# Jellyman750/Linear_Programming_Solver_LPR381

Hardware: AMD Instinct MI355X
Metric: simplex pivots/sec on dense m×n tableau; B&B nodes/sec at 1/2/4/8 GPUs (higher is better)
Workload: dtype f64

## Files before the change

### include/lpx.h

```cpp
#ifndef LPX_H
#define LPX_H

#include <stdint.h>

#ifdef __cplusplus
extern "C" {
#endif

#define LPX_ABI_VERSION 1

enum {
    LPX_OPTIMAL    = 0,
    LPX_UNBOUNDED  = 1,
    LPX_INFEASIBLE = 2,
    LPX_ITER_LIMIT = 3,
    LPX_RUNNING    = 4,
    LPX_CUTOFF     = 5,
    LPX_CUT_INTEGER     = 0,
    LPX_CUT_INCOMPLETE  = 10,
    LPX_CUT_ERROR       = 11,
    LPX_CUT_NOT_OPTIMAL = 12,
    LPX_EINVAL     = -1,
    LPX_EDEVICE    = -2,
    LPX_ENOMEM     = -3,
    LPX_E_GE_PRESENT      = -10,
    LPX_E_NEG_RHS         = -11,
    LPX_E_REVISED_PRECOND = -12,
    LPX_E_SINGULAR        = -13,
    LPX_E_KNAP_SHAPE      = -14,
    LPX_E_UNKNOWN_ALGO    = -15,
    LPX_E_PARSE           = -16
};

typedef void (*lpx_pivot_cb)(void* user, int iter, int row, int col);

typedef struct lpx_stats {
    int64_t pivots;
    int64_t launches;
    double  loop_ms;
    double  h2d_ms;
    double  d2h_ms;
    double  update_ms_sum;
    int64_t update_launches;
    int64_t fdf_pivots;
    int64_t cleanup_pivots;
} lpx_stats;

typedef struct lpx_run_opts {
    double eps;
    double ratio_tol;
    int    max_iter;
    int    fdf_guard;
    int    cleanup;
    int    batch;
    int    use_graph;
    int    profile;
    int    resident;
} lpx_run_opts;

void lpx_default_opts(lpx_run_opts* o, int dual);

int         lpx_abi_version(void);
int         lpx_device_count(void);
int         lpx_init(int device);
int         lpx_last_error(char* buf, int len);
int         lpx_device_name(char* buf, int len);

#define LPX_COMM_ID_BYTES 128
int lpx_comm_unique_id(uint8_t* id );
int lpx_comm_init(int rank, int world, const uint8_t* id);
int lpx_comm_init_tcp(int rank, int world, const char* host, int port);
int lpx_comm_allreduce_max(double* vals, int count);
int lpx_comm_info(int* rank, int* world, int64_t* allreduces, double* allreduce_ms, int* rccl_version);
int lpx_comm_destroy(void);

typedef struct lpx_tableau lpx_tableau;

int  lpx_tableau_create(int R, int C, lpx_tableau** out);
void lpx_tableau_destroy(lpx_tableau* t);
int  lpx_tableau_upload(lpx_tableau* t, const double* T, const int32_t* basis );
int  lpx_tableau_download(lpx_tableau* t, double* T, int32_t* basis );
int  lpx_tableau_snapshot(lpx_tableau* t);
int  lpx_tableau_restore(lpx_tableau* t);
int  lpx_tableau_device_ptr(lpx_tableau* t, void** dptr, int* ld);
int  lpx_tableau_trace(lpx_tableau* t, int32_t* trace , int cap, int* n);
int  lpx_tableau_shape(const lpx_tableau* t, int* R, int* C, int* ld);
int  lpx_tableau_set_shape(lpx_tableau* t, int R, int C);


int lpx_primal_run(lpx_tableau* t, const lpx_run_opts* o, lpx_pivot_cb cb, void* user, lpx_stats* st);

int lpx_dual_run(lpx_tableau* t, const lpx_run_opts* o, lpx_pivot_cb cb, void* user, lpx_stats* st);

int lpx_forced_pivots_run(lpx_tableau* t, const int32_t* rows, const int32_t* cols, int count,
                          double thresh, int32_t* chosen, const lpx_run_opts* o, lpx_stats* st);

int lpx_tableau_solution(lpx_tableau* t, int nvars, double* x, double* z);

int lpx_tableau_build_node(lpx_tableau* node, const lpx_tableau* root, int ncuts, const int32_t* var,
                           const double* coef, const double* zero, const double* rhs);

int lpx_tableau_build_nodes(lpx_tableau** nodes, const lpx_tableau* root, int count, const int32_t* cut_off,
                            const int32_t* var, const double* coef, const double* zero, const double* rhs);

int lpx_tableau_build_child(lpx_tableau* child, lpx_tableau* parent, int var, int row_of_var, int is_ge, double bound);
int lpx_tableau_basis(lpx_tableau* t, int32_t* basis );
int lpx_tableau_solution2(lpx_tableau* t, int nvars, double* x, double* z, int32_t* basis_out );
int lpx_multi_solution(lpx_tableau** ts, int count, int nvars, double* x, double* z, int32_t* basis_out, int basis_stride);
typedef struct lpx_store lpx_store;
int  lpx_store_create(int Rcap, int Ccap, lpx_store** out);
void lpx_store_destroy(lpx_store* s);
int  lpx_store_save(lpx_store* s, lpx_tableau* t, int* slot_out);
int  lpx_store_release(lpx_store* s, int slot);
int  lpx_store_save_multi(lpx_store** stores, lpx_tableau** ts, int count, int* slots);
int  lpx_tableau_build_child_from_store(lpx_tableau* child, lpx_store* s, int slot, int var, int row_of_var,
                                        int is_ge, double bound);

int  lpx_tableau_build_children_from_store(lpx_tableau** children, lpx_store** stores, const int* slots, int count,
                                           const int32_t* var, const int32_t* row_of_var, const int32_t* is_ge, const double* bound);

int lpx_multi_run(lpx_tableau** ts, const int* dual, int count, const lpx_run_opts* primal_opts,
                  const lpx_run_opts* dual_opts, int* statuses, lpx_stats* stats );

int lpx_multi_run_some(lpx_tableau** ts, const int* dual, int count, const lpx_run_opts* primal_opts,
                       const lpx_run_opts* dual_opts, int* statuses, lpx_stats* stats , int min_active);

#define LPX_ASYNC_SLOTS 4
int lpx_multi_run_begin(int slot, lpx_tableau** ts, const int* dual, int count, const lpx_run_opts* primal_opts,
                        const lpx_run_opts* dual_opts, int steps);
int lpx_multi_run_end(int slot, int* statuses, lpx_stats* stats );

int lpx_primal_tableau(double* T, int R, int C, int32_t* basis, double eps, int max_iter,
                       lpx_pivot_cb cb, void* user, lpx_stats* st);
int lpx_dual_tableau(double* T, int R, int C, int32_t* basis, double eps, double ratio_tol,
                     int fdf_guard, int max_iter, int cleanup,
                     lpx_pivot_cb cb, void* user, lpx_stats* st);

typedef struct lpx_revised lpx_revised;
int  lpx_revised_create(int m, int n, const double* A, const double* c, const double* b, lpx_revised** out);
void lpx_revised_destroy(lpx_revised* r);
int  lpx_revised_run(lpx_revised* r, const lpx_run_opts* o, lpx_pivot_cb cb, void* user, lpx_stats* st);
int  lpx_revised_result(lpx_revised* r, int32_t* Bidx, int32_t* Nidx, double* xB, double* z);
int  lpx_revised_binv(lpx_revised* r, double* Binv );
int  lpx_revised_iteration_view(lpx_revised* r, double* rc, double* d);
int  lpx_revised_refactor(lpx_revised* r);
int  lpx_revised_set_refactor(lpx_revised* r, int every);
int  lpx_revised_set_refactor_mode(lpx_revised* r, int mode);
int  lpx_revised_set_drift_policy(lpx_revised* r, int check_every, double tol);
int  lpx_revised_residual(lpx_revised* r, double* rel , double* abs_ );
int  lpx_revised_refactor_stats(lpx_revised* r, int* refactors, int* fast_steps, int* fast_fallbacks, double* last_residual,
                                double* gemm_ms, int* gemm_calls);
int  lpx_revised_profile(lpx_revised* r, int iters, double* us , int* measured);
int  lpx_invert(const double* M, int n, double* inv);
int  lpx_invert_blocked(const double* M, int n, double* inv, double* ms);
int  lpx_revised_trace(lpx_revised* r, int32_t* trace , int cap, int* n);
int  lpx_revised_solve(const double* A, int m, int n, const double* c, const double* b,
                       int32_t* Bidx, int32_t* Nidx, double* xB, double* z,
                       double eps, int max_iter, lpx_pivot_cb cb, void* user, lpx_stats* st);

typedef struct lpx_knapsack lpx_knapsack;
int  lpx_knapsack_create(const double* profit, const double* weight, int n, double cap, lpx_knapsack** out);
void lpx_knapsack_destroy(lpx_knapsack* k);
int  lpx_knapsack_order(lpx_knapsack* k, int32_t* order );
int  lpx_knapsack_relax_batch(lpx_knapsack* k, int count, const int32_t* off, const int32_t* fix_idx,
                              const int8_t* fix_val, double* profit, double* weight, int32_t* frac_idx,
                              double* frac_val);
int  lpx_knapsack_relax_batch2(lpx_knapsack* k, int count, const int32_t* off, const int32_t* fix_idx,
                               const int8_t* fix_val, double* profit, double* weight, int32_t* frac_idx,
                               double* frac_val);
int  lpx_knapsack_has_prefix(lpx_knapsack* k);
int  lpx_knapsack_expand_batch(lpx_knapsack* k, int count, const int64_t* parent, const int32_t* item, const int8_t* val,
                               int64_t* child, double* profit, double* weight, int32_t* frac_idx, double* frac_val);
int  lpx_knapsack_expand_begin(lpx_knapsack* k, int count, const int64_t* parent, const int32_t* item, const int8_t* val, int64_t* child);
int  lpx_knapsack_expand_finish(lpx_knapsack* k, double* profit, double* weight, int32_t* frac_idx, double* frac_val);
int  lpx_knapsack_node_list(lpx_knapsack* k, int64_t node, int32_t* idx, int8_t* val, int cap, int* depth);

enum { LPX_MAX = 0, LPX_MIN = 1 };
enum { LPX_LE = 0, LPX_GE = 1, LPX_EQ = 2 };

typedef struct lpx_problem {
    int sense, n, m;
    const double* c;
    const double* A;
    const int32_t* rel;
    const double* b;
} lpx_problem;

typedef struct lpx_solve_opts {
    int max_iter;
    int batch;
    int render_iterations;
    int dual_flags;
    int bnb_mode;
    int bnb_search;
    int concurrent_nodes;
    int rank, world;
    int64_t max_nodes;
    void (*allreduce_max)(void* user, double* vals, int count);
    void* allreduce_user;
    void (*text_cb)(void* user, const char* text, const uint8_t* highlight, int R, int C);
    void* text_user;
    int bnb_dive;
} lpx_solve_opts;

typedef struct lpx_result {
    int status;
    int has_solution;
    double optimal_value;
    int n; double* x;
    int R, C; double* T;
    int32_t* basis;
    int n_pivots; int32_t* trace;
    char* report; char* summary;
    int64_t lp_solves, nodes;
    int n_log; int32_t* node_log;
    double* node_z;
    double aux[4];
    lpx_stats stats;
    int n_cuts; double* cuts;
} lpx_result;

void lpx_default_solve_opts(lpx_solve_opts* o);
int  lpx_solve(const lpx_problem* p, const char* algorithm, const lpx_solve_opts* o, lpx_result* out);
void lpx_result_free(lpx_result* r);

typedef struct lpx_parsed { int sense, n, m; double* c; double* A; int32_t* rel; double* b; int ragged; } lpx_parsed;
int  lpx_parse_text(const char* text, lpx_parsed* out);
void lpx_parsed_free(lpx_parsed* p);
int  lpx_format_number(double v, char* buf, int len);

int lpx_sensitivity_range_report(const lpx_problem* p, const double* T, int R, int C, const int32_t* basis,
                                 const char* target, char* buf, int len);
int lpx_sensitivity_range(const lpx_problem* p, const double* T, int R, int C, const int32_t* basis,
                          const char* target, double* min, double* max);
int lpx_sensitivity_apply_change(const lpx_problem* p, const double* T, int R, int C, const int32_t* basis,
                                 const char* target, double value, int* field, int* index, char* buf, int len);
int lpx_sensitivity_shadow_prices(const lpx_problem* p, const double* T, int R, int C, const int32_t* basis,
                                  char* buf, int len);
int lpx_sensitivity_solve_duality(const lpx_problem* p, const double* T, int R, int C, const int32_t* basis,
                                  const lpx_solve_opts* o, lpx_result* out);

int lpx_tableau_ranging(lpx_tableau* t, double eps,
                        double* col_inc, int32_t* col_inc_at, double* col_dec, int32_t* col_dec_at,
                        double* row_inc, int32_t* row_inc_at, double* row_dec, int32_t* row_dec_at,
                        double* min_rhs, double* min_dj);
int lpx_tableau_ranging_pairs(lpx_tableau* t, double eps, int K, const int32_t* a, const int32_t* b,
                              double* inc, int32_t* inc_at, double* dec, int32_t* dec_at);

typedef struct lpx_ranging {
    int n, m, valid;
    double min_rhs, min_dj;
    double* cost_lo; double* cost_hi; int32_t* cost_lo_at; int32_t* cost_hi_at;
    double* reduced_cost;
    double* rhs_lo; double* rhs_hi; int32_t* rhs_lo_at; int32_t* rhs_hi_at;
    double* dual;
} lpx_ranging;
int  lpx_solve_ranging(const lpx_problem* p, const char* algorithm, const lpx_solve_opts* o, lpx_result* out, lpx_ranging* rg);
void lpx_ranging_free(lpx_ranging* rg);

typedef struct lpx_cut_opts {
    int    cuts_per_round;
    int    max_rounds;
    int    max_active;
    int    purge;
    double away, coef_eps, max_dynamism, purge_tol, int_tol;
} lpx_cut_opts;
void lpx_default_cut_opts(lpx_cut_opts* o);
int  lpx_tableau_gmi_round(lpx_tableau* t, const uint8_t* is_int, int n_mask, int first_cut_col,
                           const lpx_cut_opts* o, int* n_added, int32_t* src_rows ,
                           int* n_purged, int32_t* purged_cols );
int  lpx_solve_cuts(const lpx_problem* p, const lpx_solve_opts* o, const lpx_cut_opts* co, lpx_result* out);

#define LPX_POSTOPT_SEG 64
int lpx_tableau_rhs_update(lpx_tableau* t, int K, const int32_t* cols, const double* v);
int lpx_tableau_objective_update(lpx_tableau* t, int K, const int32_t* rows, const double* w, int Kd, const int32_t* dcols,
                                 const double* dd);
int lpx_tableau_add_column(lpx_tableau* t, int K, const int32_t* cols, const double* v, double obj);
int lpx_tableau_add_row(lpx_tableau* t, int K, const int32_t* rows, const double* w, const double* base );

typedef struct lpx_session lpx_session;
typedef struct lpx_session_opts {
    int extra_rows;
    int extra_cols;
    int max_iter;
    int batch;
    int want_tableau;
} lpx_session_opts;
void lpx_default_session_opts(lpx_session_opts* o);
int  lpx_session_open(const lpx_problem* p, const lpx_session_opts* o, lpx_session** s, lpx_result* res);
int  lpx_session_set_rhs(lpx_session* s, int K, const int32_t* cons, const double* b, lpx_result* res);
int  lpx_session_set_cost(lpx_session* s, int K, const int32_t* vars, const double* c, lpx_result* res);
int  lpx_session_add_variable(lpx_session* s, double c, const double* a , lpx_result* res);
int  lpx_session_add_constraint(lpx_session* s, const double* a , int rel, double b, lpx_result* res);
int  lpx_session_ranging(lpx_session* s, lpx_ranging* rg);
int  lpx_session_shape(const lpx_session* s, int* n_vars, int* n_cons);
void lpx_session_close(lpx_session* s);

int lpx_tableau_set_bounds(lpx_tableau* t, int ncols, const double* ub);
int lpx_tableau_bound_flags(lpx_tableau* t, uint8_t* flip );
int lpx_bounded_run(lpx_tableau* t, const lpx_run_opts* o, lpx_pivot_cb cb, void* user, lpx_stats* st);
int lpx_bounded_counts(lpx_tableau* t, int64_t counts[3]);
int lpx_tableau_bounded_solution(lpx_tableau* t, int nvars, double* x, double* z, uint8_t* at_upper );

typedef struct lpx_bounded_info {
    int ncols, n;
    uint8_t* flip;
    double* ub;
    double* lower;
} lpx_bounded_info;
int  lpx_solve_bounded(const lpx_problem* p, const double* lower , const double* upper ,
                       const lpx_solve_opts* o, lpx_result* out, lpx_bounded_info* info );
void lpx_bounded_info_free(lpx_bounded_info* info);

int lpx_tableau_bound_state(lpx_tableau* t, double* lo , double* ub , uint8_t* flip );
int lpx_tableau_change_bounds(lpx_tableau* t, int K, const int32_t* cols, const double* lower, const double* upper);
int lpx_bounded_dual_run(lpx_tableau* t, const lpx_run_opts* o, lpx_pivot_cb cb, void* user, lpx_stats* st);

typedef struct lpx_bounded_session lpx_bounded_session;
int  lpx_bounded_open(const lpx_problem* p, const double* lower , const double* upper ,
                      const lpx_solve_opts* o, lpx_bounded_session** session, lpx_result* res);
int  lpx_bounded_set_bounds(lpx_bounded_session* s, int K, const int32_t* vars, const double* lower, const double* upper,
                            lpx_result* res);
void lpx_bounded_close(lpx_bounded_session* s);

#define LPX_BDUAL_SKIP_FIXED 1
typedef struct lpx_branch_pick {
    int32_t var;
    int32_t candidates;
    double x_var;
    double z;
} lpx_branch_pick;
typedef struct lpx_node_record {
    int32_t status;
    int32_t events;
    int64_t kind0, kind1;
    int64_t flips;
    int64_t unrepairable;
    lpx_branch_pick pick;
} lpx_node_record;
int lpx_tableau_dualize(lpx_tableau* t, double eps, int64_t counts[2]);
int lpx_bounded_dual_run2(lpx_tableau* t, const lpx_run_opts* o, int flags, lpx_pivot_cb cb, void* user, lpx_stats* st);
int lpx_tableau_branch_pick(lpx_tableau* t, int nint, const uint8_t* is_int , double tol, lpx_branch_pick* out);
int lpx_bounded_node(lpx_tableau* t, int K, const int32_t* cols, const double* lower, const double* upper, const lpx_run_opts* o,
                     int nint, const uint8_t* is_int , double tol, lpx_node_record* out);

typedef struct lpx_bnb_node_log {
    int32_t depth, K, status, events, flips, var;
    double z;
} lpx_bnb_node_log;
typedef struct lpx_bnb_bounded_info {
    int64_t nodes, events, flips, incumbents, pruned_bound, pruned_infeasible, max_K;
    double constant;
    int64_t n_log;
    lpx_bnb_node_log* log;
} lpx_bnb_bounded_info;
int  lpx_solve_bnb_bounded(const lpx_problem* p, const double* lower , const double* upper ,
                           const uint8_t* is_int , const lpx_solve_opts* o, int64_t max_nodes ,
                           lpx_result* out, lpx_bnb_bounded_info* info );
void lpx_bnb_bounded_info_free(lpx_bnb_bounded_info* info);

#define LPX_BDUAL_LONG_STEP 2
#define LPX_BDUAL_CUTOFF 4
int lpx_bounded_dual_run3(lpx_tableau* t, const lpx_run_opts* o, int flags, double cutoff, lpx_pivot_cb cb, void* user, lpx_stats* st);
int lpx_bounded_node2(lpx_tableau* t, int K, const int32_t* cols, const double* lower, const double* upper, const lpx_run_opts* o,
                      int flags, double cutoff, int nint, const uint8_t* is_int , double tol,
                      lpx_node_record* out);
int lpx_solve_bnb_bounded2(const lpx_problem* p, const double* lower , const double* upper ,
                           const uint8_t* is_int , const lpx_solve_opts* o, int64_t max_nodes ,
                           int search_flags, lpx_result* out, lpx_bnb_bounded_info* info );
int lpx_solve_bounded_dual(const lpx_problem* p, const double* lower , const double* upper ,
                           int flags, const lpx_solve_opts* o, lpx_result* out, lpx_bounded_info* info );

#define LPX_NODE_LAUNCHES 0
#define LPX_NODE_ONCHIP 1
#define LPX_NODE_AUTO 2
int lpx_bounded_node_fits(int R, int C);
int lpx_bounded_node3(lpx_tableau* t, int K, const int32_t* cols, const double* lower, const double* upper, const lpx_run_opts* o,
                      int flags, double cutoff, int nint, const uint8_t* is_int , double tol,
                      int form, lpx_node_record* out);
int lpx_solve_bnb_bounded3(const lpx_problem* p, const double* lower , const double* upper ,
                           const uint8_t* is_int , const lpx_solve_opts* o, int64_t max_nodes ,
                           int search_flags, int node_form, lpx_result* out, lpx_bnb_bounded_info* info );

typedef struct lpx_node_batch lpx_node_batch;
typedef struct lpx_bnb_divers_info {
    int64_t rounds, steals, largest_batch;
    int32_t* round;
    int32_t* diver;
} lpx_bnb_divers_info;
int  lpx_tableau_clone(const lpx_tableau* src, lpx_tableau** out);
int  lpx_node_batch_create(int W, lpx_tableau* const* handles, lpx_node_batch** out);
void lpx_node_batch_destroy(lpx_node_batch* b);
int  lpx_node_batch_run(lpx_node_batch* b, int B, const int32_t* slot , const int32_t* K ,
                        const int32_t* cols, const double* lower, const double* upper ,
                        const lpx_run_opts* o, int flags, const double* cutoff ,
                        int nint, const uint8_t* is_int , double tol,
                        lpx_node_record* out , int32_t* rc );
int  lpx_solve_bnb_bounded4(const lpx_problem* p, const double* lower , const double* upper ,
                            const uint8_t* is_int , const lpx_solve_opts* o, int64_t max_nodes ,
                            int search_flags, int divers , lpx_result* out, lpx_bnb_bounded_info* info ,
                            lpx_bnb_divers_info* dinfo );
void lpx_bnb_divers_info_free(lpx_bnb_divers_info* dinfo);

typedef struct lpx_bnb_plunge_info {
    int64_t launched, dropped, longest_chain;
    int32_t* step;
} lpx_bnb_plunge_info;
int  lpx_node_batch_plunge(lpx_node_batch* b, int B, const int32_t* slot , const int32_t* K ,
                           const int32_t* cols, const double* lower, const double* upper ,
                           const lpx_run_opts* o, int flags, const double* cutoff ,
                           const double* prune , const int32_t* depth , int D,
                           int nint, const uint8_t* is_int , double tol,
                           lpx_node_record* out , int32_t* steps , int32_t* rc );
int  lpx_solve_bnb_bounded5(const lpx_problem* p, const double* lower , const double* upper ,
                            const uint8_t* is_int , const lpx_solve_opts* o, int64_t max_nodes ,
                            int search_flags, int divers , int plunge , lpx_result* out,
                            lpx_bnb_bounded_info* info , lpx_bnb_divers_info* dinfo ,
                            lpx_bnb_plunge_info* pinfo );
void lpx_bnb_plunge_info_free(lpx_bnb_plunge_info* pinfo);

#define LPX_PROBE_NONE (-2)
#define LPX_BRANCH_MOST_FRACTIONAL 0
#define LPX_BRANCH_STRONG 1
typedef struct lpx_probe_head {
    int32_t count;
    int32_t candidates;
    double z;
} lpx_probe_head;
typedef struct lpx_probe_record {
    int32_t status;
    int32_t events, kind0, kind1;
    int32_t flips;
    int32_t var, dir;
    int32_t pad;
    double x_var;
    double lower, upper;
    double z;
} lpx_probe_record;
typedef struct lpx_bnb_strong_info {
    int64_t probe_launches, probes, probe_events, probe_limit, pruned_by_probe, changed_picks;
} lpx_bnb_strong_info;
int  lpx_bounded_probe(lpx_tableau* t, const lpx_run_opts* o, int flags, double cutoff, double prune,
                       int nint, const uint8_t* is_int , double tol, int cand_max ,
                       int probe_iter, lpx_probe_head* head, lpx_probe_record* out );
int  lpx_node_batch_run_probe(lpx_node_batch* b, int B, const int32_t* slot , const int32_t* K ,
                              const int32_t* cols, const double* lower, const double* upper ,
                              const lpx_run_opts* o, int flags, const double* cutoff ,
                              const double* prune , int nint, const uint8_t* is_int , double tol,
                              int cand_max , int probe_iter, lpx_node_record* out , lpx_probe_head* head ,
                              lpx_probe_record* probes , int32_t* rc );
int  lpx_solve_bnb_bounded6(const lpx_problem* p, const double* lower , const double* upper ,
                            const uint8_t* is_int , const lpx_solve_opts* o, int64_t max_nodes ,
                            int search_flags, int divers , int branching, int cand_max , int probe_iter,
                            lpx_result* out, lpx_bnb_bounded_info* info , lpx_bnb_divers_info* dinfo ,
                            lpx_bnb_strong_info* sinfo );
void lpx_bnb_strong_info_free(lpx_bnb_strong_info* sinfo);

typedef struct lpx_guard_record {
    int32_t bland_events;
    int32_t first_bland;
} lpx_guard_record;
typedef struct lpx_bnb_guard_info {
    int64_t guarded_nodes, bland_events, max_events;
} lpx_bnb_guard_info;
int  lpx_bounded_node4(lpx_tableau* t, int K, const int32_t* cols, const double* lower, const double* upper, const lpx_run_opts* o,
                       int flags, double cutoff, int stall_events, int nint, const uint8_t* is_int , double tol,
                       int form, lpx_node_record* out, lpx_guard_record* guard );
int  lpx_node_batch_run2(lpx_node_batch* b, int B, const int32_t* slot , const int32_t* K ,
                         const int32_t* cols, const double* lower, const double* upper ,
                         const lpx_run_opts* o, int flags, const double* cutoff ,
                         int stall_events, int nint, const uint8_t* is_int , double tol,
                         lpx_node_record* out , lpx_guard_record* guard , int32_t* rc );
int  lpx_solve_bnb_bounded7(const lpx_problem* p, const double* lower , const double* upper ,
                            const uint8_t* is_int , const lpx_solve_opts* o, int64_t max_nodes ,
                            int search_flags, int divers , int stall_events, lpx_result* out,
                            lpx_bnb_bounded_info* info , lpx_bnb_divers_info* dinfo ,
                            lpx_bnb_guard_info* ginfo );

typedef struct lpx_primal_record {
    int32_t status;
    int32_t events;
    int64_t kind0, kind1;
    int64_t flips;
    double  z;
} lpx_primal_record;
int  lpx_bounded_run2(lpx_tableau* t, const lpx_run_opts* o, int form, lpx_pivot_cb cb, void* user, lpx_stats* st);
int  lpx_node_batch_primal(lpx_node_batch* b, int B, const int32_t* slot , const lpx_run_opts* o,
                           lpx_primal_record* out , int32_t* rc );

int  lpx_solve_bounded2(const lpx_problem* p, const double* lower , const double* upper ,
                        const lpx_solve_opts* o, int form, lpx_result* out, lpx_bounded_info* info );
int  lpx_solve_bounded_batch(int count, const lpx_problem* const* problems, const double* const* lowers ,
                             const double* const* uppers , const lpx_solve_opts* o, lpx_result* outs ,
                             lpx_bounded_info* infos );
int  lpx_solve_bnb_bounded8(const lpx_problem* p, const double* lower , const double* upper ,
                            const uint8_t* is_int , const lpx_solve_opts* o, int64_t max_nodes ,
                            int search_flags, int divers , int stall_events, int root_form, lpx_result* out,
                            lpx_bnb_bounded_info* info , lpx_bnb_divers_info* dinfo ,
                            lpx_bnb_guard_info* ginfo );

typedef struct lpx_packed_models {
    int32_t count, m, n, sense;
    const double *c, *A, *b;
    const double *lower, *upper;
    int64_t c_stride, A_stride, b_stride, lower_stride, upper_stride;
} lpx_packed_models;
typedef struct lpx_packed_results {
    int32_t* status;  double* x;  double* value;
    lpx_primal_record* rec;  int32_t* basis;  uint8_t* at_upper;
} lpx_packed_results;
int lpx_packed_fits(int m, int n);
int lpx_solve_packed(const lpx_packed_models* in, const lpx_run_opts* o , const lpx_packed_results* out,
                     lpx_stats* st );

#define LPX_CUTLOOP_INTEGRAL   0
#define LPX_CUTLOOP_STALLED    1
#define LPX_CUTLOOP_ROUNDS     2
#define LPX_CUTLOOP_INFEASIBLE 3
#define LPX_CUTLOOP_ITER_LIMIT 4
#define LPX_CUTLOOP_STATUS     5
typedef struct lpx_cut_loop_record {
    int32_t rounds, added, purged, stop;
    int32_t status, R, C, pad;
    int64_t events;
    lpx_branch_pick pick;
    double* z_before;
    double* z_after;
} lpx_cut_loop_record;
int  lpx_tableau_gmi_round_bounded(lpx_tableau* t, const uint8_t* is_int, int n_mask, int first_cut_col,
                                   const lpx_cut_opts* o, int* n_added, int32_t* src_rows ,
                                   int* n_purged, int32_t* purged_cols );
int  lpx_bounded_cut_loop(lpx_tableau* t, const uint8_t* is_int, int n_mask, int first_cut_col, int nint,
                          const uint8_t* node_is_int , const lpx_cut_opts* co, const lpx_run_opts* ro ,
                          int flags, int form, lpx_cut_loop_record* rec);

typedef struct lpx_bnb_cut_info {
    int32_t ran, spare, rounds, added, purged, stop, status, R, C, n_z;
    int64_t events;
    double* z_before; double* z_after;
} lpx_bnb_cut_info;
int  lpx_solve_bnb_bounded9(const lpx_problem* p, const double* lower , const double* upper ,
                            const uint8_t* is_int , const lpx_solve_opts* o, int64_t max_nodes ,
                            int search_flags, int divers , int stall_events, int root_form,
                            const lpx_cut_opts* root_cuts , lpx_result* out, lpx_bnb_bounded_info* info ,
                            lpx_bnb_divers_info* dinfo , lpx_bnb_guard_info* ginfo ,
                            lpx_bnb_cut_info* cinfo );
void lpx_bnb_cut_info_free(lpx_bnb_cut_info* cinfo);

typedef struct lpx_fix_list {
    int32_t cap;
    int32_t n;
    int32_t* cols;
    double* lower;
    double* upper;
} lpx_fix_list;
typedef struct lpx_bnb_fix_info {
    int64_t tightened_nodes, tightened_cols, max_per_node;
} lpx_bnb_fix_info;
int  lpx_bounded_node5(lpx_tableau* t, int K, const int32_t* cols, const double* lower, const double* upper, const lpx_run_opts* o,
                       int flags, double cutoff, int stall_events, double fix_bound, int nint,
                       const uint8_t* is_int , double tol, int form, lpx_node_record* out,
                       lpx_guard_record* guard , lpx_fix_list* fix );
int  lpx_node_batch_run3(lpx_node_batch* b, int B, const int32_t* slot , const int32_t* K ,
                         const int32_t* cols, const double* lower, const double* upper ,
                         const lpx_run_opts* o, int flags, const double* cutoff ,
                         int stall_events, const double* fix_bound , int nint,
                         const uint8_t* is_int , double tol, lpx_node_record* out ,
                         lpx_guard_record* guard , lpx_fix_list* fix , int32_t* rc );
int  lpx_solve_bnb_bounded10(const lpx_problem* p, const double* lower , const double* upper ,
                             const uint8_t* is_int , const lpx_solve_opts* o, int64_t max_nodes ,
                             int search_flags, int divers , int stall_events, int root_form,
                             const lpx_cut_opts* root_cuts , int tighten , lpx_result* out,
                             lpx_bnb_bounded_info* info , lpx_bnb_divers_info* dinfo ,
                             lpx_bnb_guard_info* ginfo , lpx_bnb_cut_info* cinfo ,
                             lpx_bnb_fix_info* finfo );

#ifdef __cplusplus
}
#endif
#endif
```

### linear_programming_solver_lpr381_amd/csrc/lpx_handle.h

```cpp
#pragma once
#include "lpx_internal.h"

#include <cstring>

struct lpx_tableau {
    int R = 0, C = 0, ld = 0;
    int Rcap = 0, Ccap = 0;
    char* slab = nullptr;
    char* hslab = nullptr;
    int32_t* shape = nullptr;
    int32_t* shape_h = nullptr;
    double* T = nullptr;
    double* snapT = nullptr;
    double* prow = nullptr;
    double* pcol = nullptr;
    double* col0 = nullptr;
    double* col1 = nullptr;
    double* rhsbuf = nullptr;
    double* ws = nullptr;
    double* part_v = nullptr; int32_t* part_i = nullptr;
    lpx::DevState* us = nullptr;
    int32_t* basis = nullptr;
    int32_t* snapBasis = nullptr;
    int32_t* trace = nullptr;
    int trace_cap = 0;
    lpx::DevState* st = nullptr;
    lpx::DevState* hst = nullptr;
    bool suspended = false;
    bool trace_void = false;
    int32_t* frows = nullptr; int32_t* fcols = nullptr; int32_t* fchosen = nullptr; int fcap = 0;
    char* cutbuf = nullptr; char* cutbuf_h = nullptr; int cutcap = 0;
    hipStream_t stream = nullptr;
    hipGraphExec_t gexec = nullptr;
    int g_batch = 0;
    std::string g_key;
    std::vector<hipEvent_t> events;
    unsigned long long* xr = nullptr; unsigned long long* xp = nullptr; unsigned* xgen = nullptr;
    int32_t* xbasis = nullptr;
    double* xT = nullptr;
    unsigned long long* xc = nullptr; unsigned long long* xq = nullptr;
    size_t xc_bytes = 0, xq_bytes = 0;
    bool resident_off = false;
    double* fT = nullptr; char* fslab = nullptr;
    double* fprow = nullptr; double* frhs = nullptr; lpx::DevState* frec = nullptr;
    double* frat = nullptr;
    char* dring = nullptr; int dring_slots = 0;
    bool fused_off = false;
    bool suspended2 = false;
    bool fsuspended = false; int frec_cur = 0;
    char* rgws = nullptr; size_t rgws_bytes = 0;
    struct __attribute__((visibility("hidden"))) Bounds {
        double* ub = nullptr; uint8_t* flip = nullptr;
        bool bounds_set = false; int bounds_C = 0;
        double* snapUb = nullptr; uint8_t* snapFlip = nullptr; bool snap_bounds = false; int snap_bounds_C = 0;
        int64_t bcounts[3] = {0, 0, 0};
        double* lo = nullptr; double* snapLo = nullptr;
        bool lo_used = false, snap_lo_used = false;
        char* chg = nullptr; size_t chg_bytes = 0;
        int32_t* dzl = nullptr; lpx_branch_pick* pickrec = nullptr; uint8_t* pickmask = nullptr; char* nodeslab = nullptr;
        double* cutoff = nullptr; double cutoff_h = 0.0;
        char* nodeio = nullptr; size_t nodeio_bytes = 0;
        std::vector<uint8_t> mask_h; int mask_n = -1;
        std::vector<uint8_t> whole, snap_whole;
        char* probews = nullptr; size_t probews_bytes = 0;
        char* probeio = nullptr; size_t probeio_bytes = 0;

        void free()
        {
            hipFree(probews); if (probeio) hipHostFree(probeio);
            hipFree(ub); hipFree(flip); hipFree(snapUb); hipFree(snapFlip);
            hipFree(lo); hipFree(snapLo); hipFree(chg);
            hipFree(dzl); hipFree(pickrec); hipFree(pickmask); if (nodeslab) hipHostFree(nodeslab); hipFree(cutoff);
            if (nodeio) hipHostFree(nodeio);
        }
    } bnd;
};

#pragma GCC visibility push(hidden)
namespace lpx {

int bounds_snapshot(lpx_tableau* t);
int bounds_restore(lpx_tableau* t);
int bounds_clone(const lpx_tableau* src, lpx_tableau* dst);

int check_change_args(lpx_tableau* t, int K, const int32_t* cols, const double* lower, const double* upper, const char* what);
int check_pick_args(lpx_tableau* t, int nint, double tol, const void* out, const char* what);
int check_long_flags(int flags, double cutoff, const char* what);
int check_node_opts(const lpx_tableau* t, const lpx_run_opts* o, const char* what);
int check_node_fits(const lpx_tableau* t, const char* what);
int bounded_node_ready(const char* what);
void node_onchip_commit(lpx_tableau* t, const NodeOut* rec, bool any_lo, lpx_node_record* out);
void bounds_note_edit(lpx_tableau* t, int K, const int32_t* cols, const double* lower, const double* upper);
int bounded_plunge_ready(const char* what);
int bounded_guard_ready(const char* what);
int bounded_fix_ready(const char* what);
int check_fix_args(double fix_bound, const lpx_fix_list* fix, int nint, const char* what);
size_t fix_list_bytes(int nint);
void fix_list_place(char* at, int nint, FixParams* p);
void fix_commit(lpx_tableau* t, int n, const FixParams& p, lpx_fix_list* fix);
int bounded_probe_ready(const char* what);
int check_probe_args(int cand_max, int probe_iter, const char* what);
size_t probe_ws_bytes(const lpx_tableau* t, int cand_max);
void probe_params(const lpx_tableau* t, const lpx_run_opts* o, int flags, double cutoff, double prune, int nint, const uint8_t* mask_dev,
                  double tol, int cand_max, int probe_iter, bool lo_used, char* ws, const NodeOut* front, lpx_probe_head* head,
                  lpx_probe_record* rec, ProbeParams* p);
int bounded_primal_ready(const char* what);
int bounded_primal_prepare(lpx_tableau* t);
void primal_params(lpx_tableau* t, const lpx_run_opts* o, lpx_primal_record* rec, PrimalParams* n);
void primal_onchip_commit(lpx_tableau* t, const lpx_primal_record* rec);

static constexpr int LPX_RESIDENT_RETRY = -1000;

void drop_graph(lpx_tableau* t);
bool fused_buffers(lpx_tableau* t);
SelParams base_params(lpx_tableau* t, const lpx_run_opts* o, int mode);

inline DevState fresh_state(bool dual)
{
    DevState init; std::memset(&init, 0, sizeof(init));
    init.status = LPX_RUNNING; init.r = -1; init.q = -1; init.qn = -1; init.phase = dual ? 0 : 2;
    return init;
}
inline void resume_from(DevState& init, const DevState& at, bool dual)
{
    init.iter = at.iter; init.phase = dual ? at.phase : 2;
    init.fdf_count = at.fdf_count; init.dual_iter = at.dual_iter; init.primal_count = at.primal_count;
}
inline long long pivot_budget(const lpx_run_opts* o, bool dual)
{
    return dual ? (long long)o->fdf_guard + 2LL * o->max_iter : (long long)o->max_iter;
}
inline void stats_from_state(lpx_stats& s, const DevState& d, bool dual, double loop_ms, long long launches, bool keep_transfers)
{
    const double h2d = s.h2d_ms, d2h = s.d2h_ms;
    std::memset(&s, 0, sizeof(s));
    if (keep_transfers) { s.h2d_ms = h2d; s.d2h_ms = d2h; }
    s.pivots = d.iter; s.fdf_pivots = d.fdf_count;
    s.cleanup_pivots = dual ? d.primal_count : 0;
    s.loop_ms = loop_ms; s.launches = launches;
}

template <typename Params, typename Enqueue>
void make_ctx(lpx_tableau* t, const SelParams& p, const Params& key, Enqueue enqueue, LoopCtx& c, DevState& init)
{
    const bool lookahead = p.mode != MODE_DUAL && p.mode != MODE_BOUNDED;
    c.stream = t->stream; c.st = t->st; c.hst = t->hst; c.trace = t->trace; c.trace_cap = t->trace_cap;
    t->trace_void = false;
    c.events = &t->events; c.gexec = &t->gexec; c.g_batch = &t->g_batch; c.g_key = &t->g_key;
    c.key.assign(reinterpret_cast<const char*>(&key), sizeof(key));
    c.enqueue_iter = enqueue;
    if (lookahead)
        c.prologue = [p](hipStream_t s) -> int { LPX_HIP_TRY(launch_la_init(p, s)); return 0; };
    else
        c.prologue = [p](hipStream_t s) -> int { LPX_HIP_TRY(launch_rhs_init(p, s)); return 0; };
    c.launches_per_iter = 2;
    c.profile_maps = lookahead;
    init = fresh_state(p.mode == MODE_DUAL);
}
void make_ctx(lpx_tableau* t, const SelParams& p, LoopCtx& c, DevState& init);
int run_loop(lpx_tableau* t, SelParams p, const lpx_run_opts* o, long long budget,
             lpx_pivot_cb cb, void* user, lpx_stats* stats, int start_iter = 0);
int continue_streaming(lpx_tableau* t, const lpx_run_opts* o, bool dual, const DevState& at, lpx_pivot_cb cb, void* user, lpx_stats* st);

int run_resident(lpx_tableau* t, const lpx_run_opts* o, lpx_pivot_cb cb, void* user, lpx_stats* stats,
                 int grid, int rpw, size_t lds, int* resume_iter, bool col = false);
struct ResGroupPlan { int grid = 0, slots = 0; size_t lds = 0; int nt = 0, rt = 0; };
ResGroupPlan resident_group_plan(lpx_tableau** ts, int count);
int run_resident_group(lpx_tableau** ts, const int* dual, int count, const lpx_run_opts* popts, const lpx_run_opts* dopts,
                       int* statuses, lpx_stats* stats, const ResGroupPlan& plan, lpx_pivot_cb cb, void* user,
                       DevState* resume = nullptr);
int multi_run_fused(lpx_tableau** ts, const int* dual, int count, const lpx_run_opts* popts, const lpx_run_opts* dopts,
                    int* statuses, lpx_stats* stats, const DevState* inits, int min_active);

}
#pragma GCC visibility pop
```

### linear_programming_solver_lpr381_amd/csrc/lpx_internal.h

```cpp
#pragma once
#include <hip/hip_runtime.h>
#include <stdint.h>
#include <string>
#include <vector>
#include <functional>
#include "../../include/lpx.h"

namespace lpx {

struct DevState {
    int status;
    int iter;
    int r, q;
    int phase;
    int fdf_count;
    int dual_iter;
    int primal_count;
    int forced_k;
    int qn;
    int c0n;
    int qn_valid;
    int pad[4];
};

enum { MODE_PRIMAL = 0, MODE_DUAL = 1, MODE_FORCED = 2, MODE_BOUNDED = 3 };

struct SelParams {
    double* T; int ld; int R; int C;
    const int32_t* shape;
    double* prow;
    double* pcol;
    double* col0;
    double* col1;
    double* rhsbuf;
    int32_t* basis;
    int32_t* trace;
    int trace_cap;
    DevState* st;
    DevState* us;
    double* part_v; int32_t* part_i; int nblk;
    int qsel;
    double eps;
    double tol_fdf;
    double tol_dual;
    double tol_primal;
    int max_iter, fdf_guard, cleanup, mode;
    const int32_t* frows; const int32_t* fcols; int fcount; double fthresh; int32_t* fchosen;
    double* ws;
    int rcap;
};

struct BndParams {
    SelParams P;
    const double* ub;
    uint8_t* flip;
    int dual;
    const double* cutoff;
};
hipError_t launch_bounded_select(const BndParams& b, hipStream_t s);
hipError_t launch_bounded_dual_select(const BndParams& b, hipStream_t s);

hipError_t launch_dualize_list(const double* T, int ld, int R, int Cm, const double* ub, double eps, int32_t* list, int32_t* cnt,
                               hipStream_t s);
hipError_t launch_dualize_apply(double* T, int ld, int R, int Cm, const double* ub, uint8_t* flip, const int32_t* list,
                                const int32_t* cnt, double* rhsbuf, hipStream_t s);
hipError_t launch_bounds_save(int K, const int32_t* cols, double* ub, double* lo, double* save, int restore, hipStream_t s);
hipError_t launch_bounds_shift(int K, const int32_t* cols, const double* lower, const double* upper, double* ub, double* lo,
                               const uint8_t* flip, double* shift, hipStream_t s);
hipError_t launch_bounds_apply(double* T, int ld, int R, int Cm, int K, const int32_t* cols, const double* shift, double* rhsbuf,
                               hipStream_t s);
struct PickParams {
    const double* T; int ld, R, Cm;
    const int32_t* basis; const double* ub; const uint8_t* flip; const double* lo;
    int nint; const uint8_t* is_int; double tol;
    double* ws;
    lpx_branch_pick* out;
};
hipError_t launch_branch_pick(const PickParams& p, hipStream_t s);

struct NodeIn {
    int32_t K, flags, nint, has_mask, max_iter, lo_used;
    int32_t stall_events, pad;
    double eps, ratio_tol, cutoff, tol;
};
static_assert(sizeof(NodeIn) == 64, "the arrays behind the header start on a double");
struct NodeOut {
    int32_t status, events, kind0, kind1, flips, unrepairable, inf_k, var, candidates, pad;
    double x_var, z;
};
struct NodeParams {
    double* T; int ld, R, C;
    double* rhsbuf; int32_t* basis; int32_t* trace; int trace_cap; DevState* st;
    double* ub; double* lo; uint8_t* flip;
    double* edit;
    const uint8_t* mask;
    const NodeIn* in; NodeOut* out;
};
size_t bounded_node_lds_bytes(int R, int C);
int bounded_node_fits(int R, int C);
hipError_t bounded_node_init();
hipError_t launch_bounded_node_onchip(const NodeParams& n, hipStream_t s);
hipError_t launch_bounded_nodes_onchip(const NodeParams* P, int B, size_t lds, hipStream_t s);
struct GuardOut { NodeOut o; int32_t bland_events, first_bland; };
static_assert(sizeof(GuardOut) == 64, "the node record and the guard record share one 64-byte slot");
hipError_t bounded_guard_init();
hipError_t launch_bounded_guard_onchip(const NodeParams* P, int B, size_t lds, hipStream_t s);
struct FixParams { NodeParams n; double fix_bound; int32_t* cols; double* lower; double* upper; };
hipError_t bounded_fix_init();
hipError_t launch_bounded_fix_onchip(const FixParams* P, int B, size_t lds, hipStream_t s);
struct PlungeParams { NodeParams n; double prune; int32_t* steps; int32_t depth, pad; };
hipError_t bounded_plunge_init();
hipError_t launch_bounded_plunge_onchip(const PlungeParams* P, int B, size_t lds, hipStream_t s);
struct ProbeParams {
    const double* T; int ld, R, C;
    const int32_t* basis; const DevState* st;
    const double* ub; const double* lo; const uint8_t* flip;
    const uint8_t* mask;
    const NodeOut* front;
    int32_t* wbasis; uint8_t* wflip; int32_t wbasis_stride, wflip_stride;
    lpx_probe_head* head; lpx_probe_record* rec;
    double eps, ratio_tol, cutoff, tol, prune;
    int32_t flags, nint, has_mask, lo_used, probe_iter, cand_max;
};
hipError_t bounded_probe_init();
hipError_t launch_bounded_probe_onchip(const ProbeParams* P, int B, int cand_max, size_t lds, hipStream_t s);
struct PrimalParams {
    double* T; int ld, R, C;
    double* rhsbuf; int32_t* basis; int32_t* trace; int trace_cap; DevState* st;
    const double* ub; uint8_t* flip;
    double eps, ratio_tol; int32_t max_iter, pad;
    lpx_primal_record* out;
};
hipError_t bounded_primal_init();
hipError_t launch_bounded_primal_onchip(const PrimalParams& n, hipStream_t s);
hipError_t launch_bounded_primals_onchip(const PrimalParams* P, int B, size_t lds, hipStream_t s);
struct PackedParams {
    const double *c, *A, *b, *lower, *upper;
    int64_t c_stride, A_stride, b_stride, lower_stride, upper_stride;
    int32_t m, n, min, max_iter;
    double eps, ratio_tol;
    int32_t* status; double* x; double* value; lpx_primal_record* rec; int32_t* basis; uint8_t* at_upper;
    uint8_t* flip; int64_t flip_stride;
};
int packed_solve(const lpx_packed_models* in, const lpx_run_opts* o, const lpx_packed_results* out, lpx_stats* st);

hipError_t launch_select(const SelParams& p, hipStream_t s);
hipError_t launch_select_la(const SelParams& p, hipStream_t s);
hipError_t launch_la_init(const SelParams& p, hipStream_t s);
hipError_t launch_update(double* T, int ld, int R, int C, const int32_t* shape, const double* prow, double* fac0, double* fac1,
                         double* rhsbuf, const DevState* st, hipStream_t s,
                         hipEvent_t e0 = nullptr, hipEvent_t e1 = nullptr);
hipError_t launch_update(const SelParams& p, double* fac0, double* fac1, hipStream_t s, hipEvent_t e0 = nullptr, hipEvent_t e1 = nullptr);
hipError_t launch_select_mb(const SelParams& p, hipStream_t s);
hipError_t launch_update_mb(const SelParams& p, hipStream_t s, hipEvent_t e0 = nullptr, hipEvent_t e1 = nullptr);
int select_mb_blocks(int C);
hipError_t launch_group_iter(const SelParams* arr, int count, int dual, int max_nblk, int max_upd_blocks, hipStream_t s,
                             int maxR, int maxC);
hipError_t launch_group_init(const SelParams* arr, int count, hipStream_t s);
hipError_t launch_group_rhs_init(const SelParams* arr, int count, hipStream_t s);
hipError_t launch_rhs_init(const SelParams& p, hipStream_t s);
int update_blocks(int ld, int R);
int update_policy(int ld, int R);
hipError_t kernels_init();

struct BuildDesc { double* T; int32_t* basis; int32_t* shape; DevState* st; int ld, R, C, cut0; };
hipError_t launch_build_nodes(const double* T0, int ld0, int R0, int C0, const BuildDesc* descs, int count, int maxld, int maxR,
                              const int32_t* cvar, const double* ccoef, const double* czero, const double* crhs, hipStream_t s);
struct ChildDesc { const double* Tp; const int32_t* basis_p; double* T; int32_t* basis; int32_t* shape; DevState* st;
                   int ldp, Rp, Cp, ld, var, ik, is_ge, pad; double bound; };
hipError_t launch_build_children(const ChildDesc* descs, int count, int maxld, int maxR, hipStream_t s);
struct ParkDesc { const double* srcT; double* dstT; const int32_t* srcB; int32_t* dstB; size_t doubles; int m, pad; };
hipError_t launch_park_many(const ParkDesc* descs, int count, int blocks_per_node, hipStream_t s);
struct GatherDesc { const double* T; const int32_t* basis; int ld, R, C, off; };
hipError_t launch_gather_solution(const GatherDesc* descs, int count, double* out_rhs, int32_t* out_basis, hipStream_t s);
hipError_t launch_build_child(const double* Tp, int ldp, int Rp, int Cp, const int32_t* basis_p, double* T, int ld,
                              int var, int ik, int is_ge, double bound, int32_t* basis, hipStream_t s);
hipError_t launch_build_node(const double* T0, int ld0, int R0, int C0, double* T, int ld, int R, int C,
                             const int32_t* cvar, const double* ccoef, const double* czero, const double* crhs,
                             int32_t* basis, hipStream_t s);
hipError_t launch_states_scatter(const SelParams* arr, const DevState* src_pinned, int count, hipStream_t s);
hipError_t launch_states_gather(const SelParams* arr, DevState* dst_pinned, int count, hipStream_t s);

struct FusedParams {
    SelParams P;
    double* T1; double* prow1; double* rhs1;
    DevState* rec;
    int par;
    double* pring; double* fring; int32_t* rring;
    int defer;
    int lm;
};
int fused_policy(int ld, int R);
int pivot_defer_max();
hipError_t launch_fused_init(const FusedParams& f, hipStream_t s);
bool pivot_select_is_pair(int ld, int R);
size_t pivot_ratio_bytes(int R);
size_t pivot_stream_bytes();
hipError_t launch_pivot_fused(const FusedParams& f, double* rat, long long L, hipStream_t s, hipEvent_t e0 = nullptr, hipEvent_t e1 = nullptr);
hipError_t launch_pivot_flush(const FusedParams& f, int buf, int n, int slot0, hipStream_t s);
hipError_t pivot_fused_init();

hipError_t launch_group_fused_init(const FusedParams* arr, const int* fresh, int nfresh, const DevState* init, hipStream_t s);
hipError_t launch_group_fused_gather(const FusedParams* arr, int count, DevState* out, int* cur, hipStream_t s);
int group_fused_blocks(int ld, int R);
int group_fused_comp_ints(int cap);
int group_fused_comp_hdr();
hipError_t launch_group_fused(const FusedParams* arr, const int* live, int nlive, int per_node, int lpar, size_t live_bytes, hipStream_t s,
                              int* comp, int cap, hipEvent_t e0 = nullptr, hipEvent_t e1 = nullptr);

hipError_t launch_dgemm_mfma(const double* A, int lda, const double* B, int ldb, double* C, int ldc, const double* D, int ldd,
                             int M, int N, int K, int mode, unsigned long long* absmax, hipStream_t s);
struct IbWork {
    int n = 0, ld = 0, ncand = 0;
    double *A = nullptr, *X = nullptr, *L = nullptr, *Mr = nullptr, *prow = nullptr;
    void* cand = nullptr; int32_t *ipiv = nullptr, *perm = nullptr; int* status = nullptr;
    std::vector<hipEvent_t> events;
};
int ib_alloc(IbWork& w, int n);
void ib_free(IbWork& w);
int ib_run(IbWork& w, hipStream_t s, double* ms);
struct ResNode {
    double* T; int ld, R, C;
    int32_t* basis; int32_t* trace; int trace_cap;
    DevState* st;
    DevState* st_host;
    unsigned long long* xr;
    unsigned long long* xp;
    unsigned* xgen;
    int mcap, dual;
    double eps, tol_fdf, tol_dual, tol_primal;
    int max_iter, fdf_guard, cleanup;
};
size_t resident_group_lds(int R, int C, int ld, int grid);
hipError_t resident_group_init();
hipError_t resident_regs_init();
int resident_regs_shape(int maxC, int min_ld, int mmax, int* rpw_max);
size_t resident_regs_lds(int R, int C, int rt, int cfg);
size_t resident_regs_lds_budget();
hipError_t launch_resnode_states_scatter(const void* nodes_dev, const DevState* src_pinned, int count, hipStream_t s);
hipError_t launch_resident_regs(const void* nodes_dev, int nodes, int grid, int cfg, int rt, size_t lds, int chunk, hipStream_t s);
hipError_t launch_resident_group(const void* nodes_dev, int nodes, int grid, size_t lds, int chunk, hipStream_t s);
hipError_t resident_init();
int resident_plan(int R, int C, int ld, int* grid, int* rpw, size_t* lds);
hipError_t launch_resident_primal(double* T, int ld, int R, int C, int grid, int rpw, size_t lds, int mcap,
                                  int32_t* basis, int32_t* trace, int trace_cap, DevState* st,
                                  unsigned long long* xr, unsigned long long* xp, unsigned* xgen,
                                  double eps, double tol, int max_iter, int chunk, hipStream_t s);

hipError_t resident_col_init();
int resident_col_plan(int R, int C, int* grid, int* cpw, size_t* lds);
size_t resident_col_xc_bytes(int grid);
size_t resident_col_xq_bytes(int grid, int R);
hipError_t launch_resident_primal_col(double* T, int ld, int R, int C, int grid, int cpw, size_t lds,
                                      int32_t* basis, int32_t* trace, int trace_cap, DevState* st,
                                      unsigned long long* xc, unsigned long long* xq, unsigned* xgen,
                                      double eps, double tol, int max_iter, int chunk, hipStream_t s);

struct TableauView {
    const double* T; int ld, R, C;
    const int32_t* basis;
    hipStream_t stream;
    char** ws; size_t* ws_bytes;
};
void tableau_view(lpx_tableau* t, TableauView* v);

struct CutView {
    double* T; double* T2; int ld, R, C, Rcap, Ccap;
    int32_t* basis; DevState* st;
    hipStream_t stream;
    char** ws; size_t* ws_bytes;
};
void tableau_cut_view(lpx_tableau* t, CutView* v, bool need_second);
int check_cut_opts(const lpx_cut_opts* o, const char* what);
int check_cut_opts(const lpx_cut_opts* o, const char* what, int kmin);
struct CutBounds { double* ub; double* lo; uint8_t* flip; double* rhsbuf; };
int gmi_round_args(lpx_tableau* t, const uint8_t* is_int, int n_mask, int first_cut_col, const lpx_cut_opts* o, int kmin, const char* what);
int gmi_round_run(lpx_tableau* t, const uint8_t* is_int, int n_mask, int first_cut_col, const lpx_cut_opts* o, int* n_added,
                  int32_t* src_rows, int* n_purged, int32_t* purged_cols, const CutBounds* cb, const char* what);

void set_error(const std::string& msg);
void trim_device_caches();
hipError_t malloc_retry(void** p, size_t bytes);
int ensure_device();
double now_ms();
hipStream_t borrow_stream();

struct LoopCtx {
    hipStream_t stream = nullptr;
    DevState* st = nullptr;
    DevState* hst = nullptr;
    int32_t* trace = nullptr; int trace_cap = 0;
    std::vector<hipEvent_t>* events = nullptr;
    hipGraphExec_t* gexec = nullptr;
    int* g_batch = nullptr;
    std::string* g_key = nullptr;
    std::string key;
    std::function<int(hipStream_t, hipEvent_t, hipEvent_t)> enqueue_iter;
    std::function<int(hipStream_t)> prologue;
    int launches_per_iter = 2;
    bool profile_maps = true;
    std::function<bool(long long)> sweep_launch;
    int start_iter = 0;
};
void graph_cache_drop_owner(const void* owner);
int run_device_loop(LoopCtx& c, const DevState& init, const lpx_run_opts* o, long long budget,
                    lpx_pivot_cb cb, void* user, lpx_stats* stats);

class LoopRun {
public:
    LoopRun() = default;
    LoopRun(const LoopRun&) = delete;
    LoopRun& operator=(const LoopRun&) = delete;
    int begin(const LoopCtx& c, const DevState& init, const lpx_run_opts* o, long long budget,
              lpx_pivot_cb cb, void* user);
    int submit();
    int complete();
    bool done() const { return status_ != LPX_RUNNING || enq_ >= budget_; }
    bool may_submit() const { return enq_ < budget_; }
    int in_flight() const { return head_ - tail_; }
    int finish(lpx_stats* stats);
    ~LoopRun();
private:
    DevState* stage_ = nullptr; hipEvent_t ev_[2] = {nullptr, nullptr}; int head_ = 0, tail_ = 0;
    LoopCtx c_; lpx_run_opts o_{}; long long budget_ = 0, enq_ = 0;
    lpx_pivot_cb cb_ = nullptr; void* user_ = nullptr;
    lpx_stats local_{}; int batch_ = 64; bool graph_ = false;
    int fired_ = 0, iter_before_ = 0, status_ = LPX_RUNNING, init_phase_ = 2;
    long long batch_first_ = 0;
    double t0_ = 0;
};

}

#define LPX_HIP_TRY(expr)                                                                  \
    do {                                                                                   \
        hipError_t e_ = (expr);                                                            \
        if (e_ != hipSuccess) {                                                            \
            lpx::set_error(std::string(#expr) + ": " + hipGetErrorString(e_));             \
            return LPX_EDEVICE;                                                            \
        }                                                                                  \
    } while (0)
```

### linear_programming_solver_lpr381_amd/csrc/lpx_pivot_fused.hip

```cpp
#include <algorithm>
#include "lpx_scan.h"
#include "lpx_tile.h"

namespace lpx {

static constexpr int FP_NT = 256;

__global__ __launch_bounds__(SEL_NT) void lpx_fused_init(FusedParams F)
{
    __shared__ double s_v[SEL_NW];
    __shared__ int s_i[SEL_NW];
    const SelParams& P = F.P;
    const int R = P.shape ? P.shape[0] : P.R, C = P.shape ? P.shape[1] : P.C;
    ScanRule rule; rule.forced = 0; rule.eps = P.eps; rule.thresh = P.fthresh; rule.C = C; rule.c0 = 0;
    int qn = -1;
    if (P.st->status == LPX_RUNNING) qn = la_prepare_from_T(P, R, C, P.col0, R - 1, rule, s_v, s_i);
    if (threadIdx.x == 0) {
        DevState x = *P.st;
        x.qn = qn; x.r = -1; x.q = -1; x.pad[2] = 1; x.pad[3] = 0;
        F.rec[0] = x;
        x.pad[2] = 0;
        F.rec[1] = x;
        P.part_i[MB_CNT] = 0;
    }
}

__host__ __device__ constexpr int fp_rows(int D) { return D <= 2 ? UPDS_ROWS : 8; }
__host__ __device__ constexpr int fp_rec(int buf, int npend, int slot0) { return buf | (npend << 1) | (slot0 << 8); }
__device__ __forceinline__ int fp_slot(int lm, int n, int s, int ring) { const int k = lm - n + s; return k < 0 ? k + ring : k; }

#ifdef LPX_STAMPS
#define LPX_FS_BEGIN(on) const bool fs_on_ = (on) && blockIdx.x == 0 && threadIdx.x == 0; unsigned long long fs_acc_[13] = {0}; \
    unsigned long long fs_prev_ = __builtin_amdgcn_s_memtime(); const unsigned long long fs_rt0_ = __builtin_amdgcn_s_memrealtime();
#define LPX_FS(slot) do { if (fs_on_) { const unsigned long long n_ = __builtin_amdgcn_s_memtime(); fs_acc_[(slot)] += n_ - fs_prev_; fs_prev_ = n_; } } while (0)
#define LPX_FS_W(slot) do { if (fs_on_) { asm volatile("s_waitcnt vmcnt(0) lgkmcnt(0)" ::: "memory"); } LPX_FS(slot); } while (0)
#define LPX_FS_TRIP(trip) do { if (fs_on_) { asm volatile("s_waitcnt vmcnt(0) lgkmcnt(0)" ::: "memory"); \
    const unsigned long long n_ = __builtin_amdgcn_s_memtime(), d_ = n_ - fs_prev_; fs_prev_ = n_; fs_acc_[1] += d_; fs_acc_[9] += 1; \
    if ((trip) == 0) fs_acc_[10] += d_; else if ((trip) == 1) fs_acc_[11] += d_; else fs_acc_[12] += d_; } } while (0)
#define LPX_FS_TIE() do { if (fs_on_) fs_acc_[9] += 1; } while (0)
#define LPX_FS_END(npend) do { if (fs_on_) { _Pragma("unroll") for (int k_ = 0; k_ < 13; ++k_) lpx_g_stamps[8 + k_] += fs_acc_[k_]; \
    lpx_g_stamps[28] += __builtin_amdgcn_s_memrealtime() - fs_rt0_; lpx_g_stamps[29] += 1; lpx_g_stamps[30] += (unsigned long long)(npend); } } while (0)
#else
#define LPX_FS_BEGIN(on)
#define LPX_FS(slot) do {} while (0)
#define LPX_FS_W(slot) do {} while (0)
#define LPX_FS_TRIP(trip) do {} while (0)
#define LPX_FS_TIE() do {} while (0)
#define LPX_FS_END(npend) do {} while (0)
#endif

template <int U, int SU, int NC = 0>
__device__ __forceinline__ void fused_select(const FusedParams& F, int n_, bool sweeps)
{
    const int n = NC > 0 ? NC : n_;
    __shared__ double s_fs;
    const SelParams& P = F.P;
    const int t = threadIdx.x, b = blockIdx.x;
    const int lm = F.lm, ring = 2 * F.defer;
    const int c = lm & 1;
    LPX_FS_BEGIN(!sweeps)
    const DevState cur = F.rec[c];
    DevState* nxt = F.rec + (c ^ 1);
    const int status = cur.status, seq = cur.pad[2], buf = cur.pad[3] & 1;
    const int nbuf = sweeps ? (buf ^ 1) : buf;
    const int nsel = P.nblk;
    if (b == 0 && t == 0) *P.st = cur;
    LPX_FS_W(0);
    if (status != LPX_RUNNING) {
        if (b == 0 && t == 0) { DevState x = cur; x.pad[2] = seq + 1; *nxt = x; }
        return;
    }
    const int R = P.shape ? P.shape[0] : P.R, C = P.shape ? P.shape[1] : P.C;
    const size_t ld = (size_t)P.ld, fld = (size_t)P.R;
    const double* __restrict__ src = buf ? F.T1 : P.T;
    double* __restrict__ prown = F.pring + (size_t)lm * ld;
    double* __restrict__ facn = F.fring + (size_t)lm * fld;
    const double* __restrict__ rhsc = c ? F.rhs1 : P.rhsbuf;
    double* __restrict__ rhsn = c ? P.rhsbuf : F.rhs1;
    const int m = R - 1;
    const int iter = cur.iter, primal_count = cur.primal_count;
    const int q = cur.qn;
    int final_status = LPX_RUNNING, r = -1;
    if (primal_count >= P.max_iter) final_status = LPX_ITER_LIMIT;
    else if (q < 0) final_status = LPX_OPTIMAL;
    double fs = 0.0;
    if (final_status == LPX_RUNNING) {
        const int sn = fp_slot(lm, n, n - 1, ring);
        const int rl = n ? cur.r : -1;
        const double prhs = n ? F.pring[(size_t)sn * ld + (C - 1)] : 0.0;
        double* rat = P.ws + (size_t)b * (size_t)(P.R > P.C ? P.R : P.C);
        for (int i0 = 0; i0 < R; i0 += U * FP_NT) {
            double v[U], h[U], fl[U];
#pragma unroll
            for (int u = 0; u < U; ++u) {
                const int i = min(R - 1, i0 + u * FP_NT + t);
                v[u] = src[(size_t)i * ld + q]; h[u] = rhsc[i];
            }
            LPX_FS_TRIP(i0 / (U * FP_NT));
#pragma unroll SU
            for (int s = 0; s < n; ++s) {
                const int sl = fp_slot(lm, n, s, ring);
                const double* __restrict__ fac = F.fring + (size_t)sl * fld;
                const double pq = F.pring[(size_t)sl * ld + q];
                const int rs = s == n - 1 ? rl : F.rring[sl];
#pragma unroll
                for (int u = 0; u < U; ++u) {
                    const int i = min(R - 1, i0 + u * FP_NT + t);
                    fl[u] = fac[i];
                    const double nv = v[u] - fl[u] * pq;
                    v[u] = i == rs ? pq : nv;
                }
            }
            LPX_FS_W(2);
#pragma unroll
            for (int u = 0; u < U; ++u) {
                const int i = i0 + u * FP_NT + t;
                if (i < R) {
                    const double dn = v[u];
                    const double nm = n == 0 ? h[u] : (i == rl ? prhs : h[u] - fl[u] * prhs);
                    rat[i] = dn > P.eps ? nm / dn : __builtin_inf();
                    if (b == 0) { facn[i] = dn; rhsn[i] = nm; }
                    if (i == m) s_fs = dn;
                }
            }
            LPX_FS(3);
        }
        __syncthreads();
        LPX_FS(3);
        fs = s_fs;
        r = block_hysteresis_segments<FP_NT / 64>(m, P.tol_primal, CompactRatio{rat});
        LPX_FS(4);
        if (r < 0) final_status = LPX_UNBOUNDED;
    }
    if (final_status != LPX_RUNNING) {
        if (b == 0 && t == 0) {
            DevState x = cur;
            x.status = final_status; x.r = -1; x.q = -1; x.qn = -1; x.pad[2] = seq + 1;
            x.pad[3] = fp_rec(nbuf, sweeps ? 0 : n, fp_slot(lm, n, 0, ring));
            *nxt = x;
        }
        return;
    }

    ScanRule rule; rule.forced = 0; rule.eps = P.eps; rule.thresh = P.fthresh; rule.C = C; rule.c0 = 0;
    const int per = (C + nsel - 1) / nsel;
    const int j0 = b * per, j1 = min(C, j0 + per);
    const double* trow = src + (size_t)r * ld;
    const double* orow = src + (size_t)m * ld;
    auto pslot = [&](int s) { return fp_slot(lm, n, s, ring); };
    auto prs = [&](int s) { return s == n - 1 ? cur.r : F.rring[pslot(s)]; };
    auto pfr = [&](int s) { return F.fring[(size_t)pslot(s) * fld + r]; };
    auto pfm = [&](int s) { return F.fring[(size_t)pslot(s) * fld + m]; };
    double piv = trow[q];
    for (int s = 0; s < n; ++s) {
        const double pq = F.pring[(size_t)pslot(s) * ld + q];
        const double nv = piv - pfr(s) * pq;
        piv = r == prs(s) ? pq : nv;
    }
    LPX_FS_W(5);
    MinIdx best; rule_init(rule, best);
#pragma unroll 2
    for (int j = j0 + t; j < j1; j += FP_NT) {
        double tr = trow[j], ov = orow[j];
#pragma unroll SU
        for (int s = 0; s < n; ++s) {
            const double pc = F.pring[(size_t)pslot(s) * ld + j];
            const double nt = tr - pfr(s) * pc;
            tr = r == prs(s) ? pc : nt;
            ov = ov - pfm(s) * pc;
        }
        const double p = tr / piv;
        prown[j] = p;
        const double u = ov - fs * p;
        rule_feed(rule, best, j, u);
    }
    LPX_FS_W(6);
    best = wave_min_idx(best);
    if ((t & 63) == 0) {
        const int slot = b * (FP_NT / 64) + (t >> 6);
        __hip_atomic_store(&P.part_v[slot], best.v, __ATOMIC_RELAXED, __HIP_MEMORY_SCOPE_AGENT);
        __hip_atomic_store(&P.part_i[slot], best.i, __ATOMIC_RELAXED, __HIP_MEMORY_SCOPE_AGENT);
    }
    asm volatile("s_waitcnt vmcnt(0)" ::: "memory");
    __syncthreads();
    if (t < 64) {
        int last = 0;
        if (t == 0) last = (__hip_atomic_fetch_add(&P.part_i[MB_CNT], 1, __ATOMIC_RELAXED, __HIP_MEMORY_SCOPE_AGENT) == nsel - 1) ? 1 : 0;
        last = __builtin_amdgcn_readfirstlane(last);
        if (last) {
            MinIdx x; x.v = __builtin_inf(); x.i = INT_MAX;
            const int npart = nsel * (FP_NT / 64);
            if (t < npart) {
                x.v = __hip_atomic_load(&P.part_v[t], __ATOMIC_RELAXED, __HIP_MEMORY_SCOPE_AGENT);
                x.i = __hip_atomic_load(&P.part_i[t], __ATOMIC_RELAXED, __HIP_MEMORY_SCOPE_AGENT);
            }
            if (t + 64 < npart) {
                MinIdx y;
                y.v = __hip_atomic_load(&P.part_v[t + 64], __ATOMIC_RELAXED, __HIP_MEMORY_SCOPE_AGENT);
                y.i = __hip_atomic_load(&P.part_i[t + 64], __ATOMIC_RELAXED, __HIP_MEMORY_SCOPE_AGENT);
                x = mi_pick(x, y);
            }
            x = wave_min_idx(x);
            if (t == 0) {
                nxt->qn = (x.i == INT_MAX) ? -1 : x.i;
                __hip_atomic_store(&P.part_i[MB_CNT], 0, __ATOMIC_RELAXED, __HIP_MEMORY_SCOPE_AGENT);
            }
        }
    }
    LPX_FS_W(7);
    if (b == 0 && t == 0) {
        P.basis[r] = q;
        if (iter < P.trace_cap) { P.trace[2 * iter] = r; P.trace[2 * iter + 1] = q; }
        F.rring[lm] = r;
        nxt->status = LPX_RUNNING; nxt->iter = iter + 1; nxt->r = r; nxt->q = q;
        nxt->phase = cur.phase; nxt->fdf_count = cur.fdf_count; nxt->dual_iter = cur.dual_iter;
        nxt->primal_count = primal_count + 1; nxt->forced_k = cur.forced_k; nxt->c0n = 0; nxt->qn_valid = 0;
        nxt->pad[0] = cur.pad[0]; nxt->pad[1] = cur.pad[1]; nxt->pad[2] = seq + 1;
        nxt->pad[3] = sweeps ? fp_rec(nbuf, 1, lm) : fp_rec(nbuf, n + 1, fp_slot(lm, n, 0, ring));
    }
    LPX_FS_W(8);
    LPX_FS_END(n);
}

template <bool NT, int D, int ROWS = fp_rows(D)>
__device__ __forceinline__ void fused_sweep(const FusedParams& F, int ncw, int nunits, int mixmod)
{
    const SelParams& P = F.P;
    const int t = threadIdx.x;
    const int lm = F.lm;
    constexpr int ring = 2 * D;
    const DevState& cur = F.rec[lm & 1];
    const int status = cur.status, buf = cur.pad[3] & 1, rnew = cur.r;
    const int nsel = P.nblk;
    const int R = P.shape ? P.shape[0] : P.R;
    const size_t ld = (size_t)P.ld, fld = (size_t)P.R;
    const double* __restrict__ src = buf ? F.T1 : P.T;
    double* __restrict__ dst = buf ? P.T : F.T1;
    const int lane = t & 63;
    const int wave = __builtin_amdgcn_readfirstlane(t >> 6);
    const int unit = ((int)blockIdx.x - nsel) * (FP_NT / 64) + wave;
    if (unit >= nunits) return;
    const int cw = unit % ncw, rb = unit / ncw;
    const int col = cw * 128 + lane * 2;
    if (col >= P.ld) return;
    const int row0 = rb * ROWS;
    if (row0 >= R) return;
    bool hit = false;
#pragma unroll
    for (int s = 0; s < D; ++s) hit |= (unsigned)((s == D - 1 ? rnew : F.rring[fp_slot(lm, D, s, ring)]) - row0) < (unsigned)ROWS;
    if (status != LPX_RUNNING) return;
    const double* sb = src + (size_t)row0 * ld + col;
    double* db = dst + (size_t)row0 * ld + col;
    if (row0 + ROWS <= R && !hit) {
        double2 v[ROWS];
        tile_load<ROWS, NT>(v, sb, ld);
#pragma unroll
        for (int s = 0; s < D; ++s) {
            const int sl = fp_slot(lm, D, s, ring);
            const double2 p = *reinterpret_cast<const double2*>(F.pring + (size_t)sl * ld + col);
            tile_pivot<ROWS>(v, p, F.fring + (size_t)sl * fld + row0, 0);
        }
        tile_store<ROWS, NT, NT ? MIX_SWEEP : MIX_NONE>(db, ld, v, rb, mixmod);
        return;
    }
#pragma unroll 1
    for (int k = 0; k < ROWS; ++k) {
        const int i = row0 + k;
        if (i >= R) break;
        double2 o = upd_load<NT>(sb + (size_t)k * ld);
#pragma unroll 1
        for (int s = 0; s < D; ++s) {
            const int sl = fp_slot(lm, D, s, ring);
            const double2 p = *reinterpret_cast<const double2*>(F.pring + (size_t)sl * ld + col);
            const double f = F.fring[(size_t)sl * fld + i];
            double2 u;
            u.x = o.x - f * p.x;
            u.y = o.y - f * p.y;
            o = i == F.rring[sl] ? p : u;
        }
        upd_store<NT>(db + (size_t)k * ld, o);
    }
}

template <bool NT, int D>
__device__ __forceinline__ void fused_sweep_strip(const FusedParams& F, int ncw, int nunits, int mixmod)
{
    constexpr int ROWS = fp_rows(D), S = FP_STRIP_BLOCKS, ring = 2 * D;
    const SelParams& P = F.P;
    const int t = threadIdx.x;
    const int lm = F.lm;
    const DevState& cur = F.rec[lm & 1];
    const int status = cur.status, buf = cur.pad[3] & 1, rnew = cur.r;
    const int nsel = P.nblk;
    const int R = P.shape ? P.shape[0] : P.R;
    const size_t ld = (size_t)P.ld, fld = (size_t)P.R;
    const double* __restrict__ src = buf ? F.T1 : P.T;
    double* __restrict__ dst = buf ? P.T : F.T1;
    const int lane = t & 63;
    const int wave = __builtin_amdgcn_readfirstlane(t >> 6);
    const int unit = ((int)blockIdx.x - nsel) * (FP_NT / 64) + wave;
    if (unit >= nunits) return;
    const int cw = unit % ncw, strip = unit / ncw;
    const int col = cw * 128 + lane * 2;
    if (col >= P.ld) return;
    const int row0 = strip * (S * ROWS);
    if (row0 >= R) return;
    int rs[D];
#pragma unroll
    for (int s = 0; s < D; ++s) rs[s] = s == D - 1 ? rnew : F.rring[fp_slot(lm, D, s, ring)];
    if (status != LPX_RUNNING) return;
    double2 p[D];
#pragma unroll
    for (int s = 0; s < D; ++s) p[s] = *reinterpret_cast<const double2*>(F.pring + (size_t)fp_slot(lm, D, s, ring) * ld + col);
    const LPX_CONSTANT double* fc = (const LPX_CONSTANT double*)F.fring;
    const int nfull = min(S, (R - row0) / ROWS);
    const double* sb = src + (size_t)row0 * ld + col;
    double* db = dst + (size_t)row0 * ld + col;
#pragma unroll 1
    for (int b = 0; b < nfull; ++b) {
        const int r0 = row0 + b * ROWS;
        bool hit = false;
#pragma unroll
        for (int s = 0; s < D; ++s) hit |= (unsigned)(rs[s] - r0) < (unsigned)ROWS;
        double2 v[ROWS];
        tile_load<ROWS, NT>(v, sb, ld);
        if (!hit) {
#pragma unroll
            for (int s = 0; s < D; ++s) tile_pivot<ROWS>(v, p[s], fc + (size_t)fp_slot(lm, D, s, ring) * fld + r0, 0);
        } else {
#pragma unroll 1
            for (int s = 0; s < D; ++s) {
                const int sl = fp_slot(lm, D, s, ring);
                const double2 ps = *reinterpret_cast<const double2*>(F.pring + (size_t)sl * ld + col);
                const int r = s == D - 1 ? rnew : F.rring[sl];
                const LPX_CONSTANT double* f = fc + (size_t)sl * fld + r0;
#pragma unroll
                for (int k = 0; k < ROWS; ++k) {
                    double2 u;
                    u.x = v[k].x - f[k] * ps.x;
                    u.y = v[k].y - f[k] * ps.y;
                    v[k] = r0 + k == r ? ps : u;
                }
            }
        }
        tile_store<ROWS, NT, NT ? MIX_SWEEP : MIX_NONE>(db, ld, v, strip * S + b, mixmod);
        sb += (size_t)ROWS * ld; db += (size_t)ROWS * ld;
    }
    if (nfull == S) return;
#pragma unroll 1
    for (int i = row0 + nfull * ROWS; i < min(R, row0 + (nfull + 1) * ROWS); ++i) {
        double2 o = upd_load<NT>(src + (size_t)i * ld + col);
#pragma unroll 1
        for (int s = 0; s < D; ++s) {
            const int sl = fp_slot(lm, D, s, ring);
            const double2 ps = *reinterpret_cast<const double2*>(F.pring + (size_t)sl * ld + col);
            const double f = F.fring[(size_t)sl * fld + i];
            double2 u;
            u.x = o.x - f * ps.x;
            u.y = o.y - f * ps.y;
            o = i == F.rring[sl] ? ps : u;
        }
        upd_store<NT>(dst + (size_t)i * ld + col, o);
    }
}

__host__ __device__ constexpr int fp_strip_wpe(int D) { return D <= 2 ? 6 : 3; }
template <int D>
__global__ __launch_bounds__(FP_NT) __attribute__((amdgpu_waves_per_eu(fp_strip_wpe(D)))) void lpx_pivot_fused(FusedParams F, int ncw, int nunits, int mixmod)
{
    if ((int)blockIdx.x < F.P.nblk) {
        if (D == 1) fused_select<4, 1, 1>(F, 1, true);
        else fused_select<4, 1>(F, F.defer, true);
    } else if constexpr (D <= 2) fused_sweep<true, D>(F, ncw, nunits, mixmod);
    else fused_sweep_strip<true, D>(F, ncw, nunits, mixmod);
}
template <int D>
__global__ __launch_bounds__(FP_NT) __attribute__((amdgpu_waves_per_eu(6))) void lpx_pivot_fused_c(FusedParams F, int ncw, int nunits, int mixmod)
{
    if ((int)blockIdx.x < F.P.nblk) {
        if (D == 1) fused_select<4, 1, 1>(F, 1, true);
        else fused_select<4, 1>(F, F.defer, true);
    } else fused_sweep<false, D>(F, ncw, nunits, mixmod);
}
template <int U, int SU>
__global__ __launch_bounds__(FP_NT) void lpx_pivot_select_ws(FusedParams F)
{
    fused_select<U, SU>(F, F.lm % F.defer, false);
}


__device__ __forceinline__ double lane_f64(double x, int k)
{
    return __hiloint2double(__builtin_amdgcn_readlane(__double2hiint(x), k), __builtin_amdgcn_readlane(__double2loint(x), k));
}

#ifdef LPX_STAMPS
#define LPX_FC_BEGIN() const bool fc_on_ = blockIdx.x == 0 && threadIdx.x == 0; unsigned long long fc_acc_[3] = {0}; \
    unsigned long long fc_prev_ = __builtin_amdgcn_s_memtime(); const unsigned long long fc_rt0_ = __builtin_amdgcn_s_memrealtime();
#define LPX_FC_W(slot) do { if (fc_on_) { asm volatile("s_waitcnt vmcnt(0) lgkmcnt(0)" ::: "memory"); \
    const unsigned long long n_ = __builtin_amdgcn_s_memtime(); fc_acc_[(slot)] += n_ - fc_prev_; fc_prev_ = n_; } } while (0)
#define LPX_FC_END(npend) do { if (fc_on_) { _Pragma("unroll") for (int k_ = 0; k_ < 3; ++k_) lpx_g_stamps[21 + k_] += fc_acc_[k_]; \
    lpx_g_stamps[24] += __builtin_amdgcn_s_memrealtime() - fc_rt0_; lpx_g_stamps[25] += 1; lpx_g_stamps[26] += (unsigned long long)(npend); } } while (0)
#else
#define LPX_FC_BEGIN()
#define LPX_FC_W(slot) do {} while (0)
#define LPX_FC_END(npend) do {} while (0)
#endif

template <int N>
__device__ __forceinline__ void pivot_ratio_patch(const FusedParams& F, int c, int q)
{
    if (N >= 2 && blockIdx.x == 0 && threadIdx.x == 0) F.rec[c].qn = q;
}
struct SelcExchange { double v[SELC_ROWS / 64]; int i[SELC_ROWS / 64]; int n[SELC_ROWS / 64]; };
template <int N>
__device__ __forceinline__ void pivot_ratio_rows(const FusedParams& F, double* __restrict__ rat, SelcExchange& X)
{
    const SelParams& P = F.P;
    const int t = threadIdx.x;
    const int lm = F.lm, ring = 2 * F.defer, c = lm & 1;
    LPX_FC_BEGIN()
    int R = P.R, C = P.C;
    if (P.shape) { R = P.shape[0]; C = P.shape[1]; }
    MinIdx part; part.v = 0.0; part.i = 0;
    if (N >= 2) {
        const int k = min(t & 63, P.nblk - 1);
        part.v = P.part_v[k]; part.i = P.part_i[k];
    }
    const DevState cur = F.rec[c];
    if (N >= 2) asm volatile("" :: "s"(cur.status), "s"(cur.primal_count), "s"(cur.r), "s"(cur.pad[3]), "s"(R), "s"(C) : "memory");
    const int status = cur.status, primal_count = cur.primal_count, rnew = cur.r, buf = cur.pad[3] & 1;
    int q = cur.qn;
    if (status != LPX_RUNNING || primal_count >= P.max_iter) return;
    if (N >= 2) {
        part = wave_min_idx(part);
        q = part.i == INT_MAX ? -1 : part.i;
    }
    if (q < 0) { pivot_ratio_patch<N>(F, c, q); return; }
    if ((int)blockIdx.x * SELC_ROWS >= R) return;
    LPX_FC_W(0);
    const size_t ld = (size_t)P.ld, fld = (size_t)P.R;
    const double* __restrict__ src = buf ? F.T1 : P.T;
    double* __restrict__ facn = F.fring + (size_t)lm * fld;
    const double* __restrict__ rhsc = c ? F.rhs1 : P.rhsbuf;
    double* __restrict__ rhsn = c ? P.rhsbuf : F.rhs1;
    const int m = R - 1;
    const int i = blockIdx.x * SELC_ROWS + t;
    const int ic = min(i, m);
    const double v0 = src[(size_t)ic * ld + q], h = rhsc[ic];
    double f[N > 0 ? N : 1], pqv = 0.0, prhs = 0.0;
    int rsv = -1;
    if (N > 0) {
#pragma unroll
        for (int s = 0; s < N; ++s) f[s] = F.fring[(size_t)fp_slot(lm, N, s, ring) * fld + ic];
        prhs = F.pring[(size_t)fp_slot(lm, N, N - 1, ring) * ld + (C - 1)];
        const size_t kslot = (size_t)fp_slot(lm, N, min(t & 63, N - 1), ring);
        pqv = F.pring[kslot * ld + q];
        rsv = F.rring[kslot];
    }
    LPX_FC_W(1);
    double v = v0;
#pragma unroll
    for (int s = 0; s < N; ++s) {
        const double pq = lane_f64(pqv, s);
        const int rs = s == N - 1 ? rnew : __builtin_amdgcn_readlane(rsv, s);
        const double nv = v - f[s] * pq;
        v = ic == rs ? pq : nv;
    }
    const double dn = v;
    const double nm = N == 0 ? h : (ic == rnew ? prhs : h - f[N > 0 ? N - 1 : 0] * prhs);
    double ratio = dn > P.eps ? nm / dn : __builtin_inf();
    asm volatile("" : "+v"(ratio));
    if (i < R) {
        rat[i] = ratio;
        facn[i] = dn; rhsn[i] = nm;
        if (i == m) rat[P.R] = dn;
    }
    constexpr int NW = SELC_ROWS / 64;
    const int wave = t >> 6;
    MinIdx lmin; lmin.v = i < m ? ratio : __builtin_inf(); lmin.i = i;
    const double rt = lmin.v;
    lmin = wave_min_idx(lmin);
    if ((t & 63) == 0) { X.v[wave] = lmin.v; X.i[wave] = lmin.i; }
    __syncthreads();
    lmin.v = X.v[0]; lmin.i = X.i[0];
#pragma unroll
    for (int w = 1; w < NW; ++w) { MinIdx y; y.v = X.v[w]; y.i = X.i[w]; lmin = mi_pick(lmin, y); }
    const int inband = __popcll(__ballot(i < m && (rt - P.tol_primal) <= lmin.v));
    if ((t & 63) == 0) X.n[wave] = inband;
    __syncthreads();
    if (t == 0) {
        int alone = 0;
#pragma unroll
        for (int w = 0; w < NW; ++w) alone += X.n[w];
        SelcRec rec; rec.v = lmin.v; rec.i = alone == 1 ? lmin.i : -1; rec.pad = 0;
        reinterpret_cast<SelcRec*>(rat + selc_rec_offset(P.R))[blockIdx.x] = rec;
    }
    pivot_ratio_patch<N>(F, c, q);
    LPX_FC_W(2);
    LPX_FC_END(N);
}

__global__ __launch_bounds__(SELC_ROWS) void lpx_pivot_ratio(FusedParams F, double* __restrict__ rat)
{
    __shared__ SelcExchange X;
    switch (F.lm % F.defer) {
    case 0: pivot_ratio_rows<0>(F, rat, X); break;
    case 1: pivot_ratio_rows<1>(F, rat, X); break;
    case 2: pivot_ratio_rows<2>(F, rat, X); break;
    case 3: pivot_ratio_rows<3>(F, rat, X); break;
    case 4: pivot_ratio_rows<4>(F, rat, X); break;
    case 5: pivot_ratio_rows<5>(F, rat, X); break;
    case 6: pivot_ratio_rows<6>(F, rat, X); break;
    case 7: pivot_ratio_rows<7>(F, rat, X); break;
    case 8: pivot_ratio_rows<8>(F, rat, X); break;
    case 9: pivot_ratio_rows<9>(F, rat, X); break;
    case 10: pivot_ratio_rows<10>(F, rat, X); break;
    case 11: pivot_ratio_rows<11>(F, rat, X); break;
    case 12: pivot_ratio_rows<12>(F, rat, X); break;
    case 13: pivot_ratio_rows<13>(F, rat, X); break;
    case 14: pivot_ratio_rows<14>(F, rat, X); break;
    default: pivot_ratio_rows<SELP_PMAX>(F, rat, X); break;
    }
}
static_assert(SELP_PMAX == 15, "lpx_pivot_ratio: one case per pending count");

__global__ __launch_bounds__(SELP_NT) void lpx_pivot_select(FusedParams F, const double* __restrict__ rat, const SelcRec* recs)
{
    extern __shared__ double sp_rat[];
    __shared__ double s_v[SELP_NT / 64];
    __shared__ int s_i[SELP_NT / 64];
    const SelParams& P = F.P;
    const int t = threadIdx.x, b = blockIdx.x, lane = t & 63;
    const int lm = F.lm, ring = 2 * F.defer;
    const int n = lm % F.defer;
    const int c = lm & 1;
    LPX_FS_BEGIN(true)
    const SelcRec srec = recs[min(lane, selc_recs(P.R) - 1)];
    const double fs = rat[P.R];
    int R = P.R, C = P.C;
    if (P.shape) { R = P.shape[0]; C = P.shape[1]; }
    const DevState cur = F.rec[c];
    DevState* nxt = F.rec + (c ^ 1);
    const int nsel = P.nblk;
    const size_t ld = (size_t)P.ld, fld = (size_t)P.R;
    const int per = (P.C + nsel - 1) / nsel;
    const int j0 = b * per, j1c = min(P.C, j0 + per);
    const int jc0 = min(j0 + t, P.C - 1);
    const size_t kslot = (size_t)fp_slot(lm, n, min(lane, n - 1), ring);
    auto pslot = [&](int s) { return (size_t)fp_slot(lm, n, min(s, n - 1), ring); };
    asm volatile("" ::: "memory");
    double pc0[SELP_PMAX];
#pragma unroll
    for (int k = 0; k < SELP_SB; ++k) pc0[k] = F.pring[pslot(k) * ld + jc0];
#pragma unroll
    for (int k = SELP_SB; k < SELP_PMAX; ++k) pc0[k] = 0.0;
    if (n > SELP_SB) {
#pragma unroll
        for (int k = SELP_SB; k < SELP_PMAX; ++k) pc0[k] = F.pring[pslot(k) * ld + jc0];
    }
    const int rsv = F.rring[kslot];
    asm volatile("" :: "s"(cur.status), "s"(cur.qn), "s"(cur.pad[3]), "s"(R) : "memory");
    const int status = cur.status, seq = cur.pad[2], buf = cur.pad[3] & 1;
    if (b == 0 && t == 0) *P.st = cur;
    LPX_FS_W(0);
    if (status != LPX_RUNNING) {
        if (b == 0 && t == 0) { DevState x = cur; x.pad[2] = seq + 1; *nxt = x; }
        return;
    }
    const double* __restrict__ src = buf ? F.T1 : P.T;
    double* __restrict__ prown = F.pring + (size_t)lm * ld;
    const int m = R - 1;
    const int iter = cur.iter, primal_count = cur.primal_count;
    const int q = cur.qn;
    int final_status = LPX_RUNNING, r = -1;
    if (primal_count >= P.max_iter) final_status = LPX_ITER_LIMIT;
    else if (q < 0) final_status = LPX_OPTIMAL;
    auto prs = [&](int s) { return s == n - 1 ? cur.r : __builtin_amdgcn_readlane(rsv, s); };
    const double* __restrict__ orow = src + (size_t)m * ld;
    const int j1 = min(j1c, C);
    double pqv = 0.0, pfmv = 0.0;
    double ov0 = 0.0;
    if (final_status == LPX_RUNNING) {
        ov0 = orow[jc0];
        pqv = F.pring[kslot * ld + q];
        pfmv = F.fring[kslot * fld + m];
        asm volatile("" ::: "memory");
        const int S = selc_recs(m);
        double best = __builtin_inf();
        int tie = -1;
        MinIdx g; g.v = lane < S ? srec.v : __builtin_inf(); g.i = lane;
        const double myv = g.v;
        g = wave_min_idx(g);
        const int gi = __builtin_amdgcn_readlane(srec.i, g.i);
        if (g.v < __builtin_inf() && __popcll(__ballot((myv - P.tol_primal) <= g.v)) == 1 && gi >= 0) r = gi;
        else {
            for (int sgi = 0; sgi < S; ++sgi) {
                const double v = lane_f64(srec.v, sgi);
                if (!(v < best - P.tol_primal)) continue;
                const int i = __builtin_amdgcn_readlane(srec.i, sgi);
                if (i < 0) { tie = sgi; break; }
                best = v; r = i;
            }
        }
        LPX_FS(4);
        if (tie >= 0) {
            for (int i0 = 0; i0 < P.R; i0 += SELP_RU * SELP_NT) {
                double x[SELP_RU];
#pragma unroll
                for (int u = 0; u < SELP_RU; ++u) x[u] = rat[min(P.R, i0 + u * SELP_NT + t)];
#pragma unroll
                for (int u = 0; u < SELP_RU; ++u) {
                    const int i = i0 + u * SELP_NT + t;
                    if (i < P.R) sp_rat[i] = x[u];
                }
            }
            __syncthreads();
            LPX_FS_TIE();
            r = wave_hysteresis_argmin(m, P.tol_primal, CompactRatio{sp_rat}, tie * SELC_ROWS, best, r);
            LPX_FS(3);
        }
        if (r < 0) final_status = LPX_UNBOUNDED;
    }
    if (final_status != LPX_RUNNING) {
        if (b == 0 && t == 0) {
            DevState x = cur;
            x.status = final_status; x.r = -1; x.q = -1; x.qn = -1; x.pad[2] = seq + 1;
            x.pad[3] = fp_rec(buf, n, fp_slot(lm, n, 0, ring));
            *nxt = x;
        }
        return;
    }

    ScanRule rule; rule.forced = 0; rule.eps = P.eps; rule.thresh = P.fthresh; rule.C = C; rule.c0 = 0;
    const double* __restrict__ trow = src + (size_t)r * ld;
    const double pfrv = F.fring[kslot * fld + r];
    double piv = trow[q];
    const double tr0 = trow[jc0];
    LPX_FS(1);
    double ov1 = ov0;
#pragma unroll
    for (int k = 0; k < SELP_PMAX; ++k) {
        if (k < n) ov1 = ov1 - lane_f64(pfmv, k) * pc0[k];
    }
    asm volatile("" : "+v"(ov1));
    for (int s = 0; s < n; ++s) {
        const double pq = lane_f64(pqv, s);
        const double nv = piv - lane_f64(pfrv, s) * pq;
        piv = r == prs(s) ? pq : nv;
    }
    LPX_FS_W(5);
    MinIdx best; rule_init(rule, best);
    for (int jb = j0; jb < j1; jb += SELP_NT) {
        const int j = jb + t, jc = min(j, C - 1);
        double tr = tr0, ov = ov1, pc[SELP_PMAX];
#pragma unroll
        for (int k = 0; k < SELP_PMAX; ++k) pc[k] = pc0[k];
        if (jb != j0) {
            tr = trow[jc]; ov = orow[jc];
            if (n > 0) {
#pragma unroll
                for (int k = 0; k < SELP_SB; ++k) pc[k] = F.pring[pslot(k) * ld + jc];
            }
            if (n > SELP_SB) {
#pragma unroll
                for (int k = SELP_SB; k < SELP_PMAX; ++k) pc[k] = F.pring[pslot(k) * ld + jc];
            }
#pragma unroll
            for (int k = 0; k < SELP_PMAX; ++k) {
                if (k < n) ov = ov - lane_f64(pfmv, k) * pc[k];
            }
        }
#pragma unroll
        for (int k = 0; k < SELP_PMAX; ++k) {
            if (k < n) {
                const double nt = tr - lane_f64(pfrv, k) * pc[k];
                tr = r == prs(k) ? pc[k] : nt;
            }
        }
        if (j < j1) {
            const double p = tr / piv;
            prown[j] = p;
            const double u = ov - fs * p;
            rule_feed(rule, best, j, u);
        }
    }
    LPX_FS_W(6);
    static_assert(SELP_NT / 64 == 8, "lanes8_min_idx: one entry per wave");
    best = wave_min_idx(best);
    if (lane == 0) { s_v[t >> 6] = best.v; s_i[t >> 6] = best.i; }
    __syncthreads();
    best.v = s_v[lane & 7]; best.i = s_i[lane & 7];
    best = lanes8_min_idx(best);
    if (n >= 1 && n <= F.defer - 2) {
        if (t == 0) { P.part_v[b] = best.v; P.part_i[b] = best.i; }
    } else if (t < 64) {
        if (t == 0) {
            __hip_atomic_store(&P.part_v[b], best.v, __ATOMIC_RELAXED, __HIP_MEMORY_SCOPE_AGENT);
            __hip_atomic_store(&P.part_i[b], best.i, __ATOMIC_RELAXED, __HIP_MEMORY_SCOPE_AGENT);
        }
        asm volatile("s_waitcnt vmcnt(0)" ::: "memory");
        int last = 0;
        if (t == 0) last = (__hip_atomic_fetch_add(&P.part_i[MB_CNT], 1, __ATOMIC_RELAXED, __HIP_MEMORY_SCOPE_AGENT) == nsel - 1) ? 1 : 0;
        last = __builtin_amdgcn_readfirstlane(last);
        if (last) {
            MinIdx x; x.v = __builtin_inf(); x.i = INT_MAX;
            if (t < nsel) {
                x.v = __hip_atomic_load(&P.part_v[t], __ATOMIC_RELAXED, __HIP_MEMORY_SCOPE_AGENT);
                x.i = __hip_atomic_load(&P.part_i[t], __ATOMIC_RELAXED, __HIP_MEMORY_SCOPE_AGENT);
            }
            x = wave_min_idx(x);
            if (t == 0) {
                nxt->qn = (x.i == INT_MAX) ? -1 : x.i;
                __hip_atomic_store(&P.part_i[MB_CNT], 0, __ATOMIC_RELAXED, __HIP_MEMORY_SCOPE_AGENT);
            }
        }
    }
    LPX_FS_W(7);
    if (b == 0 && t == 0) {
        P.basis[r] = q;
        if (iter < P.trace_cap) { P.trace[2 * iter] = r; P.trace[2 * iter + 1] = q; }
        F.rring[lm] = r;
        nxt->status = LPX_RUNNING; nxt->iter = iter + 1; nxt->r = r; nxt->q = q;
        nxt->phase = cur.phase; nxt->fdf_count = cur.fdf_count; nxt->dual_iter = cur.dual_iter;
        nxt->primal_count = primal_count + 1; nxt->forced_k = cur.forced_k; nxt->c0n = 0; nxt->qn_valid = 0;
        nxt->pad[0] = cur.pad[0]; nxt->pad[1] = cur.pad[1]; nxt->pad[2] = seq + 1;
        nxt->pad[3] = fp_rec(buf, n + 1, fp_slot(lm, n, 0, ring));
    }
    LPX_FS_W(8);
    LPX_FS_END(n);
}

__global__ __launch_bounds__(256) void lpx_pivot_flush(FusedParams F, int buf, int n, int slot0)
{
    const SelParams& P = F.P;
    const int R = P.shape ? P.shape[0] : P.R;
    const int i = blockIdx.y;
    const int j = blockIdx.x * 256 + threadIdx.x;
    if (i >= R || j >= P.ld) return;
    const size_t ld = (size_t)P.ld, fld = (size_t)P.R;
    const int ring = 2 * F.defer;
    const double* src = buf ? F.T1 : P.T;
    double v = src[(size_t)i * ld + j];
    for (int s = 0; s < n; ++s) {
        const int sl = slot0 + s < ring ? slot0 + s : slot0 + s - ring;
        const double pc = F.pring[(size_t)sl * ld + j];
        const double nv = v - F.fring[(size_t)sl * fld + i] * pc;
        v = i == F.rring[sl] ? pc : nv;
    }
    P.T[(size_t)i * ld + j] = v;
}

int fused_policy(int ld, int R) { return policy_for(tableau_bytes(ld, R), FUSED_CACHED_BYTES); }

hipError_t launch_fused_init(const FusedParams& f, hipStream_t s)
{
    hipLaunchKernelGGL(lpx_fused_init, dim3(1), dim3(SEL_NT), 0, s, f);
    return hipGetLastError();
}

using FusedKernel = void (*)(FusedParams, int, int, int);
template <int... Ds> struct FusedTable {
    static constexpr FusedKernel nt[] = { lpx_pivot_fused<Ds>... };
    static constexpr FusedKernel c[] = { lpx_pivot_fused_c<Ds>... };
};
using FusedKernels = FusedTable<1, 2, 3, 4, 5, 6, 7, 8, 9, 10, 11, 12, 13, 14, 15, 16>;
static_assert(sizeof(FusedKernels::nt) / sizeof(FusedKernel) == FP_DMAX, "one sweep kernel per depth");

int pivot_defer_max() { return FP_DMAX; }

static hipError_t launch_pivot_select_ws(const FusedParams& f, hipStream_t s, hipEvent_t e0, hipEvent_t e1)
{
    return launch_k(lpx_pivot_select_ws<6, 4>, dim3(f.P.nblk), dim3(FP_NT), 0, s, e0, e1, f);
}

static hipError_t launch_pivot_select_pair(const FusedParams& f, double* rat, hipStream_t s, hipEvent_t e0, hipEvent_t e1)
{
    const dim3 gc((f.P.R + SELC_ROWS - 1) / SELC_ROWS), gr(f.P.nblk);
    const size_t lds = sizeof(double) * (size_t)f.P.R;
    const SelcRec* recs = reinterpret_cast<const SelcRec*>(rat + selc_rec_offset(f.P.R));
    if (e0 && e1) {
        hipExtLaunchKernelGGL(lpx_pivot_ratio, gc, dim3(SELC_ROWS), 0, s, e0, nullptr, 0, f, rat);
        hipExtLaunchKernelGGL(lpx_pivot_select, gr, dim3(SELP_NT), lds, s, nullptr, e1, 0, f, (const double*)rat, recs);
    } else {
        hipLaunchKernelGGL(lpx_pivot_ratio, gc, dim3(SELC_ROWS), 0, s, f, rat);
        hipLaunchKernelGGL(lpx_pivot_select, gr, dim3(SELP_NT), lds, s, f, (const double*)rat, recs);
    }
    return hipGetLastError();
}

size_t pivot_stream_bytes() { return UPD_STREAM_BYTES; }
size_t pivot_ratio_bytes(int R) { return selc_ratio_bytes(R); }
bool pivot_select_is_pair(int ld, int R) { return R <= SELP_LDS_ROWS && tableau_bytes(ld, R) > ((size_t)SELP_MIN_MB << 20); }

hipError_t launch_pivot_fused(const FusedParams& f0, double* rat, long long L, hipStream_t s, hipEvent_t e0, hipEvent_t e1)
{
    FusedParams f = f0;
    const int d = f.defer;
    if (d < 1 || d > FP_DMAX) return hipErrorInvalidValue;
    f.lm = (int)(L % (2 * d)); f.par = f.lm & 1;
    const bool sweep = L > 0 && L % d == 0;
    const int ld = f.P.ld, R = f.P.R;
    if (!sweep) {
        if (pivot_select_is_pair(ld, R)) return rat ? launch_pivot_select_pair(f, rat, s, e0, e1) : hipErrorInvalidValue;
        return launch_pivot_select_ws(f, s, e0, e1);
    }
    const int rows = fp_rows(d);
    const int pol = fused_policy(ld, R);
    const int strip = (pol != 0 && d >= 3) ? FP_STRIP_BLOCKS : 1;
    const int ncw = (ld + 127) / 128, nunits = ncw * (((R + rows - 1) / rows + strip - 1) / strip);
    const int nblocks = f.P.nblk + (nunits + (FP_NT / 64) - 1) / (FP_NT / 64);
    int mixmod = pol == 2 ? mixmod_for(tableau_bytes(ld, R)) : 0;
    if (mixmod > 1) mixmod = std::max(1, mixmod * UPDS_ROWS / rows);
    const FusedKernel kern = pol == 0 ? FusedKernels::c[d - 1] : FusedKernels::nt[d - 1];
    return launch_k(kern, dim3(nblocks), dim3(FP_NT), 0, s, e0, e1, f, ncw, nunits, mixmod);
}

hipError_t launch_pivot_flush(const FusedParams& f, int buf, int n, int slot0, hipStream_t s)
{
    const int R = f.P.R, ld = f.P.ld;
    hipLaunchKernelGGL(lpx_pivot_flush, dim3((ld + 255) / 256, R), dim3(256), 0, s, f, buf, n, slot0);
    return hipGetLastError();
}

hipError_t pivot_fused_init()
{
    return hipFuncSetAttribute(reinterpret_cast<const void*>(lpx_pivot_select), hipFuncAttributeMaxDynamicSharedMemorySize, 8 * SELP_LDS_ROWS);
}
#ifdef LPX_STAMPS
hipError_t pivot_fused_stamps(unsigned long long* acc, int clear) { return stamps_take(acc, clear); }
#endif

}
```

### linear_programming_solver_lpr381_amd/csrc/lpx_tableau.cpp

```cpp
#include "lpx_handle.h"

#include <cstdlib>
#include <cstring>
#include <memory>
#include <vector>

namespace lpx { const std::string& get_error(); extern int g_device; }

using namespace lpx;

void lpx::tableau_view(lpx_tableau* t, TableauView* v)
{
    v->T = t->T; v->ld = t->ld; v->R = t->R; v->C = t->C;
    v->basis = t->basis; v->stream = t->stream;
    v->ws = &t->rgws; v->ws_bytes = &t->rgws_bytes;
}

void lpx::tableau_cut_view(lpx_tableau* t, CutView* v, bool need_second)
{
    v->T = t->T; v->T2 = need_second && fused_buffers(t) ? t->fT : nullptr;
    v->ld = t->ld; v->R = t->R; v->C = t->C; v->Rcap = t->Rcap; v->Ccap = t->Ccap;
    v->basis = t->basis; v->st = t->st; v->stream = t->stream;
    v->ws = &t->rgws; v->ws_bytes = &t->rgws_bytes;
}

void lpx::drop_graph(lpx_tableau* t)
{
    if (t->gexec) { hipGraphExecDestroy(t->gexec); t->gexec = nullptr; t->g_batch = 0; }
    graph_cache_drop_owner(&t->gexec);
}

extern "C" {

int lpx_abi_version(void) { return LPX_ABI_VERSION; }

int lpx_device_count(void)
{
    int n = 0;
    if (hipGetDeviceCount(&n) != hipSuccess) return 0;
    return n;
}

int lpx_init(int device)
{
    int n = lpx_device_count();
    if (device < 0 || device >= n) { set_error("lpx_init: device index out of range"); return LPX_EDEVICE; }
    LPX_HIP_TRY(hipSetDevice(device));
    g_device = device;
    return ensure_device();
}

int lpx_last_error(char* buf, int len)
{
    const std::string& e = get_error();
    if (!buf || len <= 0) return (int)e.size();
    std::strncpy(buf, e.c_str(), len - 1);
    buf[len - 1] = 0;
    return (int)e.size();
}

int lpx_device_name(char* buf, int len)
{
    int rc = ensure_device();
    if (rc) return rc;
    hipDeviceProp_t prop;
    LPX_HIP_TRY(hipGetDeviceProperties(&prop, g_device));
    std::snprintf(buf, len, "%s (%s, %d CUs)", prop.name, prop.gcnArchName, prop.multiProcessorCount);
    return 0;
}

void lpx_default_opts(lpx_run_opts* o, int dual)
{
    std::memset(o, 0, sizeof(*o));
    o->eps = 1e-9;
    o->ratio_tol = dual ? 1e-12 : 1e-9;
    o->max_iter = 10000;
    o->fdf_guard = 100;
    o->cleanup = 0;
    o->batch = 0;
    static const bool no_graph = [] { const char* e = std::getenv("LPX_GRAPH"); return e && e[0] == '0'; }();
    o->use_graph = no_graph ? 0 : 1;
    o->profile = 0;
    o->resident = 0;
}

int lpx_tableau_create(int R, int C, lpx_tableau** out)
{
    if (!out || R < 1 || C < 2) { set_error("lpx_tableau_create: bad shape"); return LPX_EINVAL; }
    int rc = ensure_device();
    if (rc) return rc;
    lpx_tableau* t = new lpx_tableau();
    t->R = R; t->C = C; t->Rcap = R; t->Ccap = C; t->ld = (C + 15) / 16 * 16;
    const size_t tb = sizeof(double) * (size_t)R * t->ld;
    const int wsn = R > C ? R : C;
    t->trace_cap = 1 << 16;
    auto up = [](size_t b) { return (b + 255) & ~(size_t)255; };
    const size_t nb = R > 1 ? (size_t)R - 1 : 1;
    const size_t sz[] = { up(sizeof(double) * t->ld), up(sizeof(double) * R), up(sizeof(double) * R), up(sizeof(double) * R),
                          up(sizeof(double) * R), up(sizeof(double) * (size_t)wsn * 32), up(sizeof(double) * 192),
                          up(sizeof(int32_t) * 256), up(sizeof(DevState)), up(sizeof(int32_t) * nb),
                          up(sizeof(int32_t) * 2 * (size_t)t->trace_cap), up(sizeof(DevState)), up(sizeof(int32_t) * 2) };
    size_t total = 0;
    for (size_t b : sz) total += b;
    hipError_t e_ = malloc_retry((void**)&t->T, tb);
    if (e_ == hipSuccess) e_ = malloc_retry((void**)&t->slab, total);
    if (e_ != hipSuccess) {
        set_error(std::string("hipMalloc failed: ") + hipGetErrorString(e_));
        lpx_tableau_destroy(t);
        return e_ == hipErrorOutOfMemory ? LPX_ENOMEM : LPX_EDEVICE;
    }
    {
        char* p = t->slab; int k = 0;
        t->prow = (double*)p; p += sz[k++];
        t->pcol = (double*)p; p += sz[k++];
        t->col0 = (double*)p; p += sz[k++];
        t->col1 = (double*)p; p += sz[k++];
        t->rhsbuf = (double*)p; p += sz[k++];
        t->ws = (double*)p; p += sz[k++];
        t->part_v = (double*)p; p += sz[k++];
        t->part_i = (int32_t*)p; p += sz[k++];
        t->us = (DevState*)p; p += sz[k++];
        t->basis = (int32_t*)p; p += sz[k++];
        t->trace = (int32_t*)p; p += sz[k++];
        t->st = (DevState*)p; p += sz[k++];
        t->shape = (int32_t*)p; p += sz[k++];
    }
    if (hipHostMalloc((void**)&t->hslab, 256 + sizeof(int32_t) * 2) != hipSuccess ||
        (t->stream = borrow_stream()) == nullptr) {
        set_error("host-pinned state / stream creation failed");
        lpx_tableau_destroy(t);
        return LPX_EDEVICE;
    }
    t->hst = (DevState*)t->hslab; t->shape_h = (int32_t*)(t->hslab + 256);
    static_assert(sizeof(DevState) <= 256, "pinned slab layout");
    hipMemsetAsync(t->T, 0, tb, t->stream);
    hipMemsetAsync(t->slab, 0, total - sz[10] - sz[11] - sz[12], t->stream);
    hipMemsetAsync(t->st, 0, sizeof(DevState), t->stream);
    t->shape_h[0] = R; t->shape_h[1] = C;
    hipMemcpyAsync(t->shape, t->shape_h, sizeof(int32_t) * 2, hipMemcpyHostToDevice, t->stream);
    LPX_HIP_TRY(hipStreamSynchronize(t->stream));
    *out = t;
    return 0;
}

void lpx_tableau_destroy(lpx_tableau* t)
{
    if (!t) return;
    if (t->stream) hipStreamSynchronize(t->stream);
    drop_graph(t);
    for (hipEvent_t e : t->events) hipEventDestroy(e);
    hipFree(t->T); hipFree(t->slab); hipFree(t->snapT); hipFree(t->snapBasis);
    hipFree(t->frows); hipFree(t->fcols); hipFree(t->fchosen); hipFree(t->cutbuf);
    hipFree(t->fT); hipFree(t->fslab); hipFree(t->dring);
    hipFree(t->rgws);
    t->bnd.free();
    hipFree(t->xr); hipFree(t->xp); hipFree(t->xgen); hipFree(t->xbasis); hipFree(t->xT); hipFree(t->xc); hipFree(t->xq);
    if (t->hslab) hipHostFree(t->hslab);
    if (t->cutbuf_h) hipHostFree(t->cutbuf_h);
    delete t;
}

int lpx_tableau_clone(const lpx_tableau* src, lpx_tableau** out)
{
    if (!src || !out) { set_error("lpx_tableau_clone: null argument"); return LPX_EINVAL; }
    if (src->suspended || src->suspended2 || src->fsuspended) {
        set_error("lpx_tableau_clone: the source is in the middle of a run that lpx_multi_run_some left unfinished");
        return LPX_EINVAL;
    }
    lpx_tableau* c = nullptr;
    int rc = lpx_tableau_create(src->Rcap, src->Ccap, &c); if (rc) return rc;
    auto fail = [&](int code) { lpx_tableau_destroy(c); return code; };
    auto copy = [&]() -> int {
        LPX_HIP_TRY(hipStreamSynchronize(src->stream));
        c->R = src->R; c->C = src->C; c->shape_h[0] = src->R; c->shape_h[1] = src->C;
        LPX_HIP_TRY(hipMemcpyAsync(c->shape, c->shape_h, sizeof(int32_t) * 2, hipMemcpyHostToDevice, c->stream));
        LPX_HIP_TRY(hipMemcpyAsync(c->T, src->T, sizeof(double) * (size_t)src->R * src->ld, hipMemcpyDeviceToDevice, c->stream));
        if (src->R > 1) LPX_HIP_TRY(hipMemcpyAsync(c->basis, src->basis, sizeof(int32_t) * (src->R - 1), hipMemcpyDeviceToDevice, c->stream));
        LPX_HIP_TRY(hipMemcpyAsync(c->rhsbuf, src->rhsbuf, sizeof(double) * src->R, hipMemcpyDeviceToDevice, c->stream));
        LPX_HIP_TRY(hipMemcpyAsync(c->st, src->st, sizeof(DevState), hipMemcpyDeviceToDevice, c->stream));
        *c->hst = *src->hst;
        c->trace_void = true;
        int r = bounds_clone(src, c); if (r) return r;
        LPX_HIP_TRY(hipStreamSynchronize(c->stream));
        return 0;
    };
    rc = copy(); if (rc) return fail(rc);
    *out = c;
    return 0;
}

int lpx_tableau_shape(const lpx_tableau* t, int* R, int* C, int* ld)
{
    if (!t) return LPX_EINVAL;
    if (R) *R = t->R;
    if (C) *C = t->C;
    if (ld) *ld = t->ld;
    return 0;
}

int lpx_tableau_upload(lpx_tableau* t, const double* T, const int32_t* basis)
{
    if (!t || !T) { set_error("lpx_tableau_upload: null argument"); return LPX_EINVAL; }
    t->suspended = t->suspended2 = t->fsuspended = false;
    LPX_HIP_TRY(hipMemcpy2DAsync(t->T, sizeof(double) * t->ld, T, sizeof(double) * t->C,
                                 sizeof(double) * t->C, t->R, hipMemcpyHostToDevice, t->stream));
    if (basis && t->R > 1)
        LPX_HIP_TRY(hipMemcpyAsync(t->basis, basis, sizeof(int32_t) * (t->R - 1), hipMemcpyHostToDevice, t->stream));
    LPX_HIP_TRY(hipMemsetAsync(t->st, 0, sizeof(DevState), t->stream));
    LPX_HIP_TRY(hipStreamSynchronize(t->stream));
    return 0;
}

int lpx_tableau_download(lpx_tableau* t, double* T, int32_t* basis)
{
    if (!t) return LPX_EINVAL;
    if (T)
        LPX_HIP_TRY(hipMemcpy2DAsync(T, sizeof(double) * t->C, t->T, sizeof(double) * t->ld,
                                     sizeof(double) * t->C, t->R, hipMemcpyDeviceToHost, t->stream));
    if (basis && t->R > 1)
        LPX_HIP_TRY(hipMemcpyAsync(basis, t->basis, sizeof(int32_t) * (t->R - 1), hipMemcpyDeviceToHost, t->stream));
    LPX_HIP_TRY(hipStreamSynchronize(t->stream));
    return 0;
}

int lpx_tableau_snapshot(lpx_tableau* t)
{
    if (!t) return LPX_EINVAL;
    const size_t tb = sizeof(double) * (size_t)t->R * t->ld;
    if (!t->snapT) {
        LPX_HIP_TRY(hipMalloc((void**)&t->snapT, sizeof(double) * (size_t)t->Rcap * t->ld));
        LPX_HIP_TRY(hipMalloc((void**)&t->snapBasis, sizeof(int32_t) * (t->Rcap > 1 ? t->Rcap - 1 : 1)));
    }
    LPX_HIP_TRY(hipMemcpyAsync(t->snapT, t->T, tb, hipMemcpyDeviceToDevice, t->stream));
    LPX_HIP_TRY(hipMemcpyAsync(t->snapBasis, t->basis, sizeof(int32_t) * (t->R > 1 ? t->R - 1 : 1),
                               hipMemcpyDeviceToDevice, t->stream));
    { int rc = bounds_snapshot(t); if (rc) return rc; }
    LPX_HIP_TRY(hipStreamSynchronize(t->stream));
    return 0;
}

int lpx_tableau_restore(lpx_tableau* t)
{
    if (!t || !t->snapT) { set_error("lpx_tableau_restore: no snapshot"); return LPX_EINVAL; }
    t->suspended = t->suspended2 = t->fsuspended = false;
    const size_t tb = sizeof(double) * (size_t)t->R * t->ld;
    LPX_HIP_TRY(hipMemcpyAsync(t->T, t->snapT, tb, hipMemcpyDeviceToDevice, t->stream));
    LPX_HIP_TRY(hipMemcpyAsync(t->basis, t->snapBasis, sizeof(int32_t) * (t->R > 1 ? t->R - 1 : 1),
                               hipMemcpyDeviceToDevice, t->stream));
    { int rc = bounds_restore(t); if (rc) return rc; }
    LPX_HIP_TRY(hipMemsetAsync(t->st, 0, sizeof(DevState), t->stream));
    LPX_HIP_TRY(hipStreamSynchronize(t->stream));
    return 0;
}

int lpx_tableau_device_ptr(lpx_tableau* t, void** dptr, int* ld)
{
    if (!t) return LPX_EINVAL;
    if (dptr) *dptr = t->T;
    if (ld) *ld = t->ld;
    return 0;
}

#ifdef LPX_STAMPS
static int debug_stamps(void* src, unsigned long long* out, int n, int clear)
{
    if (!src) return LPX_EINVAL;
    LPX_HIP_TRY(hipMemcpy(out, src, sizeof(unsigned long long) * n, hipMemcpyDeviceToHost));
    if (clear) LPX_HIP_TRY(hipMemset(src, 0, sizeof(unsigned long long) * n));
    return 0;
}
int lpx_debug_resident_col(lpx_tableau* t, unsigned long long* out, int n, int clear) { return debug_stamps(t->xc ? t->xc + 2 * 256 * 2 * 2 : nullptr, out, n, clear); }
int lpx_debug_resident_group(lpx_tableau* t, unsigned long long* out, int n, int clear) { return debug_stamps(t->xp ? t->xp + 4 * ((size_t)t->ld + 8) : nullptr, out, n, clear); }
int lpx_debug_resident(lpx_tableau* t, unsigned long long* out, int n, int clear) { return debug_stamps(t->xp ? t->xp + 4 * (size_t)t->ld : nullptr, out, n, clear); }
extern "C++" { namespace lpx { hipError_t debug_copy_stamps(unsigned long long* out, int clear); } }
int lpx_debug_hs(unsigned long long* out, int clear) { LPX_HIP_TRY(lpx::debug_copy_stamps(out, clear)); return 0; }
int lpx_debug_ws(lpx_tableau* t, unsigned long long* out, int n, int clear) { return debug_stamps(t->us ? t->part_v + 128 : t->ws, out, n, clear); }
#endif

int lpx_tableau_trace(lpx_tableau* t, int32_t* trace, int cap, int* n)
{
    if (!t) return LPX_EINVAL;
    LPX_HIP_TRY(hipMemcpyAsync(t->hst, t->st, sizeof(DevState), hipMemcpyDeviceToHost, t->stream));
    LPX_HIP_TRY(hipStreamSynchronize(t->stream));
    int k = t->trace_void ? 0 : t->hst->iter;
    if (k > t->trace_cap) k = t->trace_cap;
    if (n) *n = k;
    if (trace && cap > 0) {
        int c = k < cap ? k : cap;
        if (c > 0) LPX_HIP_TRY(hipMemcpy(trace, t->trace, sizeof(int32_t) * 2 * c, hipMemcpyDeviceToHost));
    }
    return 0;
}

}

namespace {

int enqueue_pair(const SelParams& p, hipStream_t s, hipEvent_t e0 = nullptr, hipEvent_t e1 = nullptr)
{
    if (p.mode == MODE_DUAL) {
        LPX_HIP_TRY(launch_select(p, s));
        LPX_HIP_TRY(launch_update(p, p.pcol, p.pcol, s, e0, e1));
    } else if (p.us) {
        LPX_HIP_TRY(launch_select_mb(p, s));
        LPX_HIP_TRY(launch_update_mb(p, s, e0, e1));
    } else {
        LPX_HIP_TRY(launch_select_la(p, s));
        LPX_HIP_TRY(launch_update(p, p.col0, p.col1, s, e0, e1));
    }
    return 0;
}

}

void lpx::make_ctx(lpx_tableau* t, const SelParams& p, LoopCtx& c, DevState& init)
{
    make_ctx(t, p, p, [p](hipStream_t s, hipEvent_t e0, hipEvent_t e1) -> int { return enqueue_pair(p, s, e0, e1); }, c, init);
}

int lpx::run_loop(lpx_tableau* t, SelParams p, const lpx_run_opts* o, long long budget,
                  lpx_pivot_cb cb, void* user, lpx_stats* stats, int start_iter)
{
    LoopCtx c; DevState init;
    make_ctx(t, p, c, init);
    c.start_iter = start_iter;
    return run_device_loop(c, init, o, budget, cb, user, stats);
}

int lpx::continue_streaming(lpx_tableau* t, const lpx_run_opts* o, bool dual, const DevState& at, lpx_pivot_cb cb, void* user, lpx_stats* st)
{
    SelParams p = base_params(t, o, dual ? MODE_DUAL : MODE_PRIMAL);
    LoopCtx c; DevState init;
    make_ctx(t, p, c, init);
    resume_from(init, at, dual);
    return run_device_loop(c, init, o, pivot_budget(o, dual) + (dual ? 8 : 2), cb, user, st);
}

SelParams lpx::base_params(lpx_tableau* t, const lpx_run_opts* o, int mode)
{
    SelParams p; std::memset(&p, 0, sizeof(p));
    t->trace_void = false;
    p.T = t->T; p.ld = t->ld; p.R = t->Rcap; p.C = t->Ccap; p.shape = t->shape;
    p.prow = t->prow; p.pcol = t->pcol; p.col0 = t->col0; p.col1 = t->col1; p.rhsbuf = t->rhsbuf; p.basis = t->basis; p.trace = t->trace; p.trace_cap = t->trace_cap;
    p.st = t->st;
    p.eps = o->eps;
    p.tol_fdf = o->ratio_tol; p.tol_dual = o->ratio_tol;
    p.tol_primal = (mode == MODE_DUAL) ? o->eps : o->ratio_tol;
    p.max_iter = o->max_iter; p.fdf_guard = o->fdf_guard; p.cleanup = o->cleanup; p.mode = mode;
    p.ws = t->ws;
    p.rcap = 0;
    static const bool mb_env = [] { const char* e = std::getenv("LPX_SELECT_MB"); return !(e && e[0] == '0'); }();
    if (mode != MODE_DUAL && mb_env) {
        p.us = t->us; p.part_v = t->part_v; p.part_i = t->part_i; p.nblk = select_mb_blocks(t->Ccap); p.qsel = update_policy(t->ld, t->Rcap) != 0 ? 1 : 0;
    }
    return p;
}

bool lpx::fused_buffers(lpx_tableau* t)
{
    if (t->fT) return true;
    if (t->fused_off) return false;
    auto up = [](size_t b) { return (b + 255) & ~(size_t)255; };
    const size_t tb = sizeof(double) * (size_t)t->Rcap * t->ld;
    const size_t sz[] = { up(sizeof(double) * t->ld), up(sizeof(double) * t->Rcap), up(2 * sizeof(DevState)),
                          up(pivot_ratio_bytes(t->Rcap)) };
    if (malloc_retry((void**)&t->fT, tb) != hipSuccess || malloc_retry((void**)&t->fslab, sz[0] + sz[1] + sz[2] + sz[3]) != hipSuccess) {
        (void)hipGetLastError();
        hipFree(t->fT); hipFree(t->fslab);
        t->fT = nullptr; t->fslab = nullptr; t->fused_off = true;
        return false;
    }
    t->fprow = (double*)t->fslab;
    t->frhs = (double*)(t->fslab + sz[0]);
    t->frec = (DevState*)(t->fslab + sz[0] + sz[1]);
    t->frat = (double*)(t->fslab + sz[0] + sz[1] + sz[2]);
    hipMemsetAsync(t->fT, 0, tb, t->stream);
    hipMemsetAsync(t->fslab, 0, sz[0] + sz[1] + sz[2] + sz[3], t->stream);
    return true;
}

namespace {

static constexpr int PIVOT_DEFER_STREAM = 16, PIVOT_DEFER_LARGE = 12, PIVOT_DEFER_SMALL = 4;
static constexpr size_t PIVOT_DEFER_LARGE_BYTES = (size_t)64 << 20;
static int pivot_defer(int ld, int R)
{
    static const int forced = [] { const char* e = std::getenv("LPX_PIVOT_DEFER"); return e ? std::atoi(e) : 0; }();
    if (forced > 0) return std::min(forced, pivot_defer_max());
    const size_t bytes = sizeof(double) * (size_t)ld * (size_t)R;
    if (bytes > pivot_stream_bytes()) return PIVOT_DEFER_STREAM;
    return bytes > PIVOT_DEFER_LARGE_BYTES ? PIVOT_DEFER_LARGE : PIVOT_DEFER_SMALL;
}

static int defer_ring(lpx_tableau* t, int d)
{
    if (t->dring_slots >= 2 * d) return 0;
    hipFree(t->dring); t->dring = nullptr; t->dring_slots = 0;
    const size_t slots = 2 * (size_t)d;
    const size_t bytes = slots * sizeof(double) * ((size_t)t->ld + (size_t)t->Rcap) + slots * sizeof(int32_t);
    LPX_HIP_TRY(malloc_retry((void**)&t->dring, bytes));
    LPX_HIP_TRY(hipMemsetAsync(t->dring, 0, bytes, t->stream));
    t->dring_slots = (int)slots;
    return 0;
}

static int run_fused(lpx_tableau* t, const SelParams& p, const lpx_run_opts* o, lpx_stats* stats, int start_iter)
{
    const int d = pivot_defer(t->ld, t->Rcap);
    { int rc = defer_ring(t, d); if (rc) return rc; }
    FusedParams f; std::memset(&f, 0, sizeof(f));
    f.P = p; f.T1 = t->fT; f.prow1 = t->fprow; f.rhs1 = t->frhs; f.rec = t->frec;
    f.pring = (double*)t->dring;
    f.fring = f.pring + (size_t)t->dring_slots * t->ld;
    f.rring = (int32_t*)(f.fring + (size_t)t->dring_slots * t->Rcap);
    f.defer = d;
    LoopCtx c; DevState init;
    make_ctx(t, p, c, init);
    c.key.assign(reinterpret_cast<const char*>(&f), sizeof(f));
    auto count = std::make_shared<long long>(1);
    double* rat = t->frat;
    c.enqueue_iter = [f, rat, count](hipStream_t s, hipEvent_t e0, hipEvent_t e1) -> int {
        LPX_HIP_TRY(launch_pivot_fused(f, rat, *count, s, e0, e1)); ++*count; return 0; };
    c.prologue = [f, rat, count](hipStream_t s) -> int {
        LPX_HIP_TRY(launch_fused_init(f, s)); LPX_HIP_TRY(launch_pivot_fused(f, rat, 0, s)); *count = 1; return 0; };
    c.launches_per_iter = 1;
    c.sweep_launch = [d](long long k) { return (k + 1) % d == 0; };
    c.start_iter = start_iter;
    lpx_run_opts oe = *o;
    { const int b = oe.batch > 0 ? oe.batch : 64; oe.batch = (b + 2 * d - 1) / (2 * d) * (2 * d); }
    o = &oe;
    const int rc = run_device_loop(c, init, o, pivot_budget(o, false) + 4, nullptr, nullptr, stats);
    LPX_HIP_TRY(hipStreamSynchronize(t->stream));
    DevState recs[2];
    LPX_HIP_TRY(hipMemcpy(recs, t->frec, sizeof(recs), hipMemcpyDeviceToHost));
    const DevState& last = recs[1].pad[2] > recs[0].pad[2] ? recs[1] : recs[0];
    const int buf = last.pad[3] & 1, npend = (last.pad[3] >> 1) & 31, slot0 = last.pad[3] >> 8;
    if (npend > 0) {
        LPX_HIP_TRY(launch_pivot_flush(f, buf, npend, slot0, t->stream));
        LPX_HIP_TRY(hipStreamSynchronize(t->stream));
        if (stats) stats->launches += 1;
    } else if (buf == 1) {
        LPX_HIP_TRY(hipMemcpyAsync(t->T, t->fT, sizeof(double) * (size_t)t->R * t->ld, hipMemcpyDeviceToDevice, t->stream));
        LPX_HIP_TRY(hipStreamSynchronize(t->stream));
    }
    return rc;
}


}

extern "C" {

int lpx_primal_run(lpx_tableau* t, const lpx_run_opts* o, lpx_pivot_cb cb, void* user, lpx_stats* st)
{
    if (!t) { set_error("lpx_primal_run: null tableau"); return LPX_EINVAL; }
    lpx_run_opts d; if (!o) { lpx_default_opts(&d, 0); o = &d; }
    if (t->R < 2) { set_error("lpx_primal_run: tableau needs at least one constraint row"); return LPX_EINVAL; }
    static const bool res_env = [] { const char* e = std::getenv("LPX_RESIDENT"); return !(e && e[0] == '0'); }();
    int resume = 0;
    if (o->resident > 0 || (o->resident == 0 && res_env && !o->profile && (o->batch == 0 || o->batch >= 32))) {
        int grid = 0, rpw = 0; size_t lds = 0;
        static const bool col_env = [] { const char* e = std::getenv("LPX_RESIDENT_COL"); return e && e[0] == '1'; }();
        bool col = false;
        if (!t->resident_off && col_env && resident_col_plan(t->R, t->C, &grid, &rpw, &lds)) col = true;
        if (!t->resident_off && (col || resident_plan(t->R, t->C, t->ld, &grid, &rpw, &lds))) {
            const int rc = run_resident(t, o, cb, user, st, grid, rpw, lds, &resume, col);
            if (rc != LPX_RESIDENT_RETRY) return rc;
            if (o->resident > 0) return LPX_EDEVICE;
        } else
        if (o->resident > 0) { set_error("lpx_primal_run: resident = 1 but the tableau does not fit the chip's LDS"); return LPX_EINVAL; }
    }
    SelParams p = base_params(t, o, MODE_PRIMAL);
    static const bool fused_env = [] { const char* e = std::getenv("LPX_FUSED_PIVOT"); return !(e && e[0] == '0'); }();
    if (fused_env && p.us && !cb && fused_buffers(t)) return run_fused(t, p, o, st, resume);
    return run_loop(t, p, o, pivot_budget(o, false) + 2, cb, user, st, resume);
}

int lpx_dual_run(lpx_tableau* t, const lpx_run_opts* o, lpx_pivot_cb cb, void* user, lpx_stats* st)
{
    if (!t) { set_error("lpx_dual_run: null tableau"); return LPX_EINVAL; }
    lpx_run_opts d; if (!o) { lpx_default_opts(&d, 1); o = &d; }
    if (t->R < 2) { set_error("lpx_dual_run: tableau needs at least one constraint row"); return LPX_EINVAL; }
    static const bool res_env = [] { const char* e = std::getenv("LPX_RESIDENT"); return !(e && e[0] == '0'); }();
    if (o->resident > 0 || (o->resident == 0 && res_env && !o->profile && (o->batch == 0 || o->batch >= 32))) {
        int isdual = 1, status = 0;
        const ResGroupPlan plan = t->resident_off ? ResGroupPlan{} : resident_group_plan(&t, 1);
        if (plan.slots) {
            DevState resume;
            const int rc = run_resident_group(&t, &isdual, 1, o, o, &status, st, plan, cb, user, &resume);
            if (rc == 0) return status;
            if (rc != LPX_RESIDENT_RETRY) return rc;
            t->resident_off = true;
            if (o->resident > 0) return LPX_EDEVICE;
            return continue_streaming(t, o, true, resume, cb, user, st);
        } else
        if (o->resident > 0) { set_error("lpx_dual_run: resident = 1 but the tableau does not fit the chip's LDS"); return LPX_EINVAL; }
    }
    if (!cb) {
        int isdual = 1, status = 0;
        const int rc = multi_run_fused(&t, &isdual, 1, o, o, &status, st, nullptr, 0);
        if (rc != LPX_RESIDENT_RETRY) return rc ? rc : status;
    }
    SelParams p = base_params(t, o, MODE_DUAL);
    return run_loop(t, p, o, pivot_budget(o, true) + 8, cb, user, st);
}

int lpx_forced_pivots_run(lpx_tableau* t, const int32_t* rows, const int32_t* cols, int count,
                          double thresh, int32_t* chosen, const lpx_run_opts* o, lpx_stats* st)
{
    if (!t || !rows || !cols || count < 0) { set_error("lpx_forced_pivots_run: bad argument"); return LPX_EINVAL; }
    lpx_run_opts d; if (!o) { lpx_default_opts(&d, 0); o = &d; }
    for (int k = 0; k < count; ++k)
        if (rows[k] < 0 || rows[k] >= t->R || cols[k] < 0 || cols[k] >= t->C) {
            set_error("lpx_forced_pivots_run: pivot position outside the tableau"); return LPX_EINVAL;
        }
    if (count > t->fcap) {
        hipFree(t->frows); hipFree(t->fcols); hipFree(t->fchosen);
        t->frows = t->fcols = t->fchosen = nullptr; t->fcap = 0;
        LPX_HIP_TRY(hipMalloc((void**)&t->frows, sizeof(int32_t) * count));
        LPX_HIP_TRY(hipMalloc((void**)&t->fcols, sizeof(int32_t) * count));
        LPX_HIP_TRY(hipMalloc((void**)&t->fchosen, sizeof(int32_t) * count));
        t->fcap = count;
        drop_graph(t);
    }
    if (count > 0) {
        LPX_HIP_TRY(hipMemcpyAsync(t->frows, rows, sizeof(int32_t) * count, hipMemcpyHostToDevice, t->stream));
        LPX_HIP_TRY(hipMemcpyAsync(t->fcols, cols, sizeof(int32_t) * count, hipMemcpyHostToDevice, t->stream));
        LPX_HIP_TRY(hipMemsetAsync(t->fchosen, 0xff, sizeof(int32_t) * count, t->stream));
    }
    SelParams p = base_params(t, o, MODE_FORCED);
    p.frows = t->frows; p.fcols = t->fcols; p.fcount = count; p.fthresh = thresh; p.fchosen = t->fchosen;
    int rc = run_loop(t, p, o, (long long)count + 2, nullptr, nullptr, st);
    if (chosen && count > 0)
        LPX_HIP_TRY(hipMemcpy(chosen, t->fchosen, sizeof(int32_t) * count, hipMemcpyDeviceToHost));
    return rc;
}

static int one_shot(double* T, int R, int C, int32_t* basis, const lpx_run_opts* o, int dual,
                    lpx_pivot_cb cb, void* user, lpx_stats* st)
{
    if (!T || !basis) { set_error("null tableau or basis"); return LPX_EINVAL; }
    lpx_tableau* t = nullptr;
    int rc = lpx_tableau_create(R, C, &t);
    if (rc) return rc;
    double a = now_ms();
    rc = lpx_tableau_upload(t, T, basis);
    double h2d = now_ms() - a;
    if (rc) { lpx_tableau_destroy(t); return rc; }
    lpx_stats local; std::memset(&local, 0, sizeof(local));
    int status = dual ? lpx_dual_run(t, o, cb, user, &local) : lpx_primal_run(t, o, cb, user, &local);
    if (status < 0) { lpx_tableau_destroy(t); return status; }
    a = now_ms();
    rc = lpx_tableau_download(t, T, basis);
    local.d2h_ms = now_ms() - a;
    local.h2d_ms = h2d;
    lpx_tableau_destroy(t);
    if (st) *st = local;
    return rc ? rc : status;
}

int lpx_primal_tableau(double* T, int R, int C, int32_t* basis, double eps, int max_iter,
                       lpx_pivot_cb cb, void* user, lpx_stats* st)
{
    lpx_run_opts o; lpx_default_opts(&o, 0);
    o.eps = eps; o.ratio_tol = eps; o.max_iter = max_iter;
    return one_shot(T, R, C, basis, &o, 0, cb, user, st);
}

int lpx_dual_tableau(double* T, int R, int C, int32_t* basis, double eps, double ratio_tol,
                     int fdf_guard, int max_iter, int cleanup,
                     lpx_pivot_cb cb, void* user, lpx_stats* st)
{
    lpx_run_opts o; lpx_default_opts(&o, 1);
    o.eps = eps; o.ratio_tol = ratio_tol; o.fdf_guard = fdf_guard; o.max_iter = max_iter; o.cleanup = cleanup;
    return one_shot(T, R, C, basis, &o, 1, cb, user, st);
}

}
```

Baseline: 53640.

## Run fused pivot loop on a compacted tableau that drops basic columns

Adds a compact mode to the fused pivot path. On entry, a kernel gathers the nonbasic columns into a narrower tableau and tracks variable-to-slot maps. The entering and leaving columns then swap slots on device each pivot, and an exit kernel scatters the result back to the full layout. This cuts per-pivot memory traffic and arithmetic from about m+n columns to n+1 columns. The cost is extra entry/exit passes, slot bookkeeping in select and ratio, and more kernel variants.

```diff
diff --git a/include/lpx.h b/include/lpx.h
--- a/include/lpx.h
+++ b/include/lpx.h
@@ -86,6 +86,7 @@
 int  lpx_tableau_trace(lpx_tableau* t, int32_t* trace , int cap, int* n);
 int  lpx_tableau_shape(const lpx_tableau* t, int* R, int* C, int* ld);
 int  lpx_tableau_set_shape(lpx_tableau* t, int R, int C);
+int  lpx_tableau_last_run_compact(const lpx_tableau* t);
 
 
 int lpx_primal_run(lpx_tableau* t, const lpx_run_opts* o, lpx_pivot_cb cb, void* user, lpx_stats* st);
diff --git a/linear_programming_solver_lpr381_amd/csrc/lpx_handle.h b/linear_programming_solver_lpr381_amd/csrc/lpx_handle.h
--- a/linear_programming_solver_lpr381_amd/csrc/lpx_handle.h
+++ b/linear_programming_solver_lpr381_amd/csrc/lpx_handle.h
@@ -45,6 +45,8 @@
     double* fprow = nullptr; double* frhs = nullptr; lpx::DevState* frec = nullptr;
     double* frat = nullptr;
     char* dring = nullptr; int dring_slots = 0;
+    char* cslab = nullptr;
+    bool last_compact = false;
     bool fused_off = false;
     bool suspended2 = false;
     bool fsuspended = false; int frec_cur = 0;
diff --git a/linear_programming_solver_lpr381_amd/csrc/lpx_internal.h b/linear_programming_solver_lpr381_amd/csrc/lpx_internal.h
--- a/linear_programming_solver_lpr381_amd/csrc/lpx_internal.h
+++ b/linear_programming_solver_lpr381_amd/csrc/lpx_internal.h
@@ -189,11 +189,26 @@
     double* pring; double* fring; int32_t* rring;
     int defer;
     int lm;
-};
+    int compact, ld_full;
+    int32_t* slotvar;
+    int32_t* pslot;
+    int32_t* qring;
+    int32_t* caux;
+};
+struct CompactIo {
+    double* full; int ld, R, C;
+    double* comp; int cld;
+    const int32_t* basis;
+    int32_t* vmap;
+    int32_t* slotvar; int32_t* flag;
+};
+hipError_t launch_compact_entry(const CompactIo& io, int32_t* cshape, int32_t* caux, hipStream_t s);
+hipError_t launch_compact_exit(const FusedParams& f, const CompactIo& io, const double* src, int n, int slot0, hipStream_t s);
 int fused_policy(int ld, int R);
 int pivot_defer_max();
 hipError_t launch_fused_init(const FusedParams& f, hipStream_t s);
 bool pivot_select_is_pair(int ld, int R);
+bool pivot_compact_ok(int ld, int R, int d);
 size_t pivot_ratio_bytes(int R);
 size_t pivot_stream_bytes();
 hipError_t launch_pivot_fused(const FusedParams& f, double* rat, long long L, hipStream_t s, hipEvent_t e0 = nullptr, hipEvent_t e1 = nullptr);
diff --git a/linear_programming_solver_lpr381_amd/csrc/lpx_pivot_fused.hip b/linear_programming_solver_lpr381_amd/csrc/lpx_pivot_fused.hip
--- a/linear_programming_solver_lpr381_amd/csrc/lpx_pivot_fused.hip
+++ b/linear_programming_solver_lpr381_amd/csrc/lpx_pivot_fused.hip
@@ -49,7 +49,23 @@
 #define LPX_FS_END(npend) do {} while (0)
 #endif
 
-template <int U, int SU, int NC = 0>
+__device__ __forceinline__ void cm_feed(MinIdx& m, int& mslot, int j, int var, double u)
+{
+    if (u < m.v || (u == m.v && m.i != INT_MAX && var < m.i)) { m.v = u; m.i = var; mslot = j; }
+}
+__device__ __forceinline__ void cm_pick(MinIdx& a, int& aslot, MinIdx b, int bslot)
+{
+    if (b.v < a.v || (b.v == a.v && b.i < a.i)) { a = b; aslot = bslot; }
+}
+__device__ __forceinline__ MinIdx cm_wave_min(MinIdx x, int& slot)
+{
+    const MinIdx r = wave_min_idx(x);
+    const unsigned long long mk = __ballot(x.i == r.i);
+    slot = __builtin_amdgcn_readlane(slot, __ffsll((long long)mk) - 1);
+    return r;
+}
+
+template <int U, int SU, int NC = 0, bool CM = false>
 __device__ __forceinline__ void fused_select(const FusedParams& F, int n_, bool sweeps)
 {
     const int n = NC > 0 ? NC : n_;
@@ -159,6 +175,7 @@
     }
     LPX_FS_W(5);
     MinIdx best; rule_init(rule, best);
+    int bslot = -1;
 #pragma unroll 2
     for (int j = j0 + t; j < j1; j += FP_NT) {
         double tr = trow[j], ov = orow[j];
@@ -169,17 +186,35 @@
             tr = r == prs(s) ? pc : nt;
             ov = ov - pfm(s) * pc;
         }
+        if constexpr (CM) {
+            int var = F.slotvar[j];
+            if (j == q) {
+                const int lv = P.basis[r];
+                tr = 1.0; ov = 0.0;
+                P.basis[r] = var;
+                if (iter < P.trace_cap) { P.trace[2 * iter] = r; P.trace[2 * iter + 1] = var; }
+                F.slotvar[j] = lv; F.qring[lm] = q;
+                var = lv;
+            }
+            const double p = tr / piv;
+            prown[j] = p;
+            const double u = ov - fs * p;
+            if (j < C - 1) cm_feed(best, bslot, j, var, u);
+        } else {
         const double p = tr / piv;
         prown[j] = p;
         const double u = ov - fs * p;
         rule_feed(rule, best, j, u);
+        }
     }
     LPX_FS_W(6);
-    best = wave_min_idx(best);
+    if constexpr (CM) best = cm_wave_min(best, bslot);
+    else best = wave_min_idx(best);
     if ((t & 63) == 0) {
         const int slot = b * (FP_NT / 64) + (t >> 6);
         __hip_atomic_store(&P.part_v[slot], best.v, __ATOMIC_RELAXED, __HIP_MEMORY_SCOPE_AGENT);
         __hip_atomic_store(&P.part_i[slot], best.i, __ATOMIC_RELAXED, __HIP_MEMORY_SCOPE_AGENT);
+        if constexpr (CM) __hip_atomic_store(&F.pslot[slot], bslot, __ATOMIC_RELAXED, __HIP_MEMORY_SCOPE_AGENT);
     }
     asm volatile("s_waitcnt vmcnt(0)" ::: "memory");
     __syncthreads();
@@ -189,17 +224,23 @@
         last = __builtin_amdgcn_readfirstlane(last);
         if (last) {
             MinIdx x; x.v = __builtin_inf(); x.i = INT_MAX;
+            int xs = -1;
             const int npart = nsel * (FP_NT / 64);
             if (t < npart) {
                 x.v = __hip_atomic_load(&P.part_v[t], __ATOMIC_RELAXED, __HIP_MEMORY_SCOPE_AGENT);
                 x.i = __hip_atomic_load(&P.part_i[t], __ATOMIC_RELAXED, __HIP_MEMORY_SCOPE_AGENT);
+                if constexpr (CM) xs = __hip_atomic_load(&F.pslot[t], __ATOMIC_RELAXED, __HIP_MEMORY_SCOPE_AGENT);
             }
             if (t + 64 < npart) {
                 MinIdx y;
                 y.v = __hip_atomic_load(&P.part_v[t + 64], __ATOMIC_RELAXED, __HIP_MEMORY_SCOPE_AGENT);
                 y.i = __hip_atomic_load(&P.part_i[t + 64], __ATOMIC_RELAXED, __HIP_MEMORY_SCOPE_AGENT);
+                if constexpr (CM) cm_pick(x, xs, y, __hip_atomic_load(&F.pslot[t + 64], __ATOMIC_RELAXED, __HIP_MEMORY_SCOPE_AGENT));
+                else
                 x = mi_pick(x, y);
             }
+            if constexpr (CM) { x = cm_wave_min(x, xs); if (x.i != INT_MAX) x.i = xs; }
+            else
             x = wave_min_idx(x);
             if (t == 0) {
                 nxt->qn = (x.i == INT_MAX) ? -1 : x.i;
@@ -209,8 +250,10 @@
     }
     LPX_FS_W(7);
     if (b == 0 && t == 0) {
+        if constexpr (!CM) {
         P.basis[r] = q;
         if (iter < P.trace_cap) { P.trace[2 * iter] = r; P.trace[2 * iter + 1] = q; }
+        }
         F.rring[lm] = r;
         nxt->status = LPX_RUNNING; nxt->iter = iter + 1; nxt->r = r; nxt->q = q;
         nxt->phase = cur.phase; nxt->fdf_count = cur.fdf_count; nxt->dual_iter = cur.dual_iter;
@@ -375,6 +418,13 @@
     else fused_sweep_strip<true, D>(F, ncw, nunits, mixmod);
 }
 template <int D>
+__global__ __launch_bounds__(FP_NT) __attribute__((amdgpu_waves_per_eu(fp_strip_wpe(D)))) void lpx_pivot_fused_cm(FusedParams F, int ncw, int nunits, int mixmod)
+{
+    static_assert(D >= 3, "the compact form runs the strip sweeps only");
+    if ((int)blockIdx.x < F.P.nblk) fused_select<4, 1, 0, true>(F, F.defer, true);
+    else fused_sweep_strip<true, D>(F, ncw, nunits, mixmod);
+}
+template <int D>
 __global__ __launch_bounds__(FP_NT) __attribute__((amdgpu_waves_per_eu(6))) void lpx_pivot_fused_c(FusedParams F, int ncw, int nunits, int mixmod)
 {
     if ((int)blockIdx.x < F.P.nblk) {
@@ -413,7 +463,7 @@
     if (N >= 2 && blockIdx.x == 0 && threadIdx.x == 0) F.rec[c].qn = q;
 }
 struct SelcExchange { double v[SELC_ROWS / 64]; int i[SELC_ROWS / 64]; int n[SELC_ROWS / 64]; };
-template <int N>
+template <int N, bool CM = false>
 __device__ __forceinline__ void pivot_ratio_rows(const FusedParams& F, double* __restrict__ rat, SelcExchange& X)
 {
     const SelParams& P = F.P;
@@ -423,9 +473,11 @@
     int R = P.R, C = P.C;
     if (P.shape) { R = P.shape[0]; C = P.shape[1]; }
     MinIdx part; part.v = 0.0; part.i = 0;
+    int pslot = -1;
     if (N >= 2) {
         const int k = min(t & 63, P.nblk - 1);
         part.v = P.part_v[k]; part.i = P.part_i[k];
+        if constexpr (CM) pslot = F.pslot[k];
     }
     const DevState cur = F.rec[c];
     if (N >= 2) asm volatile("" :: "s"(cur.status), "s"(cur.primal_count), "s"(cur.r), "s"(cur.pad[3]), "s"(R), "s"(C) : "memory");
@@ -433,8 +485,11 @@
     int q = cur.qn;
     if (status != LPX_RUNNING || primal_count >= P.max_iter) return;
     if (N >= 2) {
+        if constexpr (CM) { part = cm_wave_min(part, pslot); q = part.i == INT_MAX ? -1 : pslot; }
+        else {
         part = wave_min_idx(part);
         q = part.i == INT_MAX ? -1 : part.i;
+        }
     }
     if (q < 0) { pivot_ratio_patch<N>(F, c, q); return; }
     if ((int)blockIdx.x * SELC_ROWS >= R) return;
@@ -447,7 +502,9 @@
     const int m = R - 1;
     const int i = blockIdx.x * SELC_ROWS + t;
     const int ic = min(i, m);
-    const double v0 = src[(size_t)ic * ld + q], h = rhsc[ic];
+    double* srcw = buf ? F.T1 : P.T;
+    double v0 = CM ? srcw[(size_t)ic * ld + q] : src[(size_t)ic * ld + q];
+    const double h = rhsc[ic];
     double f[N > 0 ? N : 1], pqv = 0.0, prhs = 0.0;
     int rsv = -1;
     if (N > 0) {
@@ -459,6 +516,10 @@
         rsv = F.rring[kslot];
     }
     LPX_FC_W(1);
+    if constexpr (CM && N == 1) {
+        if (q == cur.q) v0 = 0.0;
+        if (i < R) srcw[(size_t)i * ld + cur.q] = 0.0;
+    }
     double v = v0;
 #pragma unroll
     for (int s = 0; s < N; ++s) {
@@ -474,6 +535,7 @@
     if (i < R) {
         rat[i] = ratio;
         facn[i] = dn; rhsn[i] = nm;
+        if constexpr (CM) srcw[(size_t)i * ld + q] = 0.0;
         if (i == m) rat[P.R] = dn;
     }
     constexpr int NW = SELC_ROWS / 64;
@@ -499,6 +561,34 @@
     pivot_ratio_patch<N>(F, c, q);
     LPX_FC_W(2);
     LPX_FC_END(N);
+}
+
+template <bool CM>
+__device__ __forceinline__ void pivot_ratio_switch(const FusedParams& F, double* __restrict__ rat, SelcExchange& X)
+{
+    switch (F.lm % F.defer) {
+    case 0: pivot_ratio_rows<0, CM>(F, rat, X); break;
+    case 1: pivot_ratio_rows<1, CM>(F, rat, X); break;
+    case 2: pivot_ratio_rows<2, CM>(F, rat, X); break;
+    case 3: pivot_ratio_rows<3, CM>(F, rat, X); break;
+    case 4: pivot_ratio_rows<4, CM>(F, rat, X); break;
+    case 5: pivot_ratio_rows<5, CM>(F, rat, X); break;
+    case 6: pivot_ratio_rows<6, CM>(F, rat, X); break;
+    case 7: pivot_ratio_rows<7, CM>(F, rat, X); break;
+    case 8: pivot_ratio_rows<8, CM>(F, rat, X); break;
+    case 9: pivot_ratio_rows<9, CM>(F, rat, X); break;
+    case 10: pivot_ratio_rows<10, CM>(F, rat, X); break;
+    case 11: pivot_ratio_rows<11, CM>(F, rat, X); break;
+    case 12: pivot_ratio_rows<12, CM>(F, rat, X); break;
+    case 13: pivot_ratio_rows<13, CM>(F, rat, X); break;
+    case 14: pivot_ratio_rows<14, CM>(F, rat, X); break;
+    default: pivot_ratio_rows<SELP_PMAX, CM>(F, rat, X); break;
+    }
+}
+__global__ __launch_bounds__(SELC_ROWS) void lpx_pivot_ratio_cm(FusedParams F, double* __restrict__ rat)
+{
+    __shared__ SelcExchange X;
+    pivot_ratio_switch<true>(F, rat, X);
 }
 
 __global__ __launch_bounds__(SELC_ROWS) void lpx_pivot_ratio(FusedParams F, double* __restrict__ rat)
@@ -525,11 +615,13 @@
 }
 static_assert(SELP_PMAX == 15, "lpx_pivot_ratio: one case per pending count");
 
-__global__ __launch_bounds__(SELP_NT) void lpx_pivot_select(FusedParams F, const double* __restrict__ rat, const SelcRec* recs)
+template <bool CM>
+__device__ __forceinline__ void pivot_select_body(const FusedParams& F, const double* __restrict__ rat, const SelcRec* recs)
 {
     extern __shared__ double sp_rat[];
     __shared__ double s_v[SELP_NT / 64];
     __shared__ int s_i[SELP_NT / 64];
+    __shared__ int s_s[SELP_NT / 64];
     const SelParams& P = F.P;
     const int t = threadIdx.x, b = blockIdx.x, lane = t & 63;
     const int lm = F.lm, ring = 2 * F.defer;
@@ -560,6 +652,8 @@
         for (int k = SELP_SB; k < SELP_PMAX; ++k) pc0[k] = F.pring[pslot(k) * ld + jc0];
     }
     const int rsv = F.rring[kslot];
+    int var0 = 0;
+    if constexpr (CM) var0 = F.slotvar[jc0];
     asm volatile("" :: "s"(cur.status), "s"(cur.qn), "s"(cur.pad[3]), "s"(R) : "memory");
     const int status = cur.status, seq = cur.pad[2], buf = cur.pad[3] & 1;
     if (b == 0 && t == 0) *P.st = cur;
@@ -583,7 +677,7 @@
     double ov0 = 0.0;
     if (final_status == LPX_RUNNING) {
         ov0 = orow[jc0];
-        pqv = F.pring[kslot * ld + q];
+        if constexpr (!CM) pqv = F.pring[kslot * ld + q];
         pfmv = F.fring[kslot * fld + m];
         asm volatile("" ::: "memory");
         const int S = selc_recs(m);
@@ -628,6 +722,7 @@
             x.status = final_status; x.r = -1; x.q = -1; x.qn = -1; x.pad[2] = seq + 1;
             x.pad[3] = fp_rec(buf, n, fp_slot(lm, n, 0, ring));
             *nxt = x;
+            if constexpr (CM) { if (final_status == LPX_UNBOUNDED) { F.caux[0] = q; F.caux[1] = lm; } }
         }
         return;
     }
@@ -635,8 +730,10 @@
     ScanRule rule; rule.forced = 0; rule.eps = P.eps; rule.thresh = P.fthresh; rule.C = C; rule.c0 = 0;
     const double* __restrict__ trow = src + (size_t)r * ld;
     const double pfrv = F.fring[kslot * fld + r];
-    double piv = trow[q];
+    double piv = CM ? F.fring[(size_t)lm * fld + r] : trow[q];
     const double tr0 = trow[jc0];
+    int lv = 0;
+    if constexpr (CM) lv = P.basis[r];
     LPX_FS(1);
     double ov1 = ov0;
 #pragma unroll
@@ -644,15 +741,20 @@
         if (k < n) ov1 = ov1 - lane_f64(pfmv, k) * pc0[k];
     }
     asm volatile("" : "+v"(ov1));
+    if constexpr (!CM) {
     for (int s = 0; s < n; ++s) {
         const double pq = lane_f64(pqv, s);
         const double nv = piv - lane_f64(pfrv, s) * pq;
         piv = r == prs(s) ? pq : nv;
     }
+    }
     LPX_FS_W(5);
     MinIdx best; rule_init(rule, best);
+    int bslot = -1;
     for (int jb = j0; jb < j1; jb += SELP_NT) {
         const int j = jb + t, jc = min(j, C - 1);
+        int var = var0;
+        if constexpr (CM) { if (jb != j0) var = F.slotvar[jc]; }
         double tr = tr0, ov = ov1, pc[SELP_PMAX];
 #pragma unroll
         for (int k = 0; k < SELP_PMAX; ++k) pc[k] = pc0[k];
@@ -678,6 +780,22 @@
                 tr = r == prs(k) ? pc[k] : nt;
             }
         }
+        if constexpr (CM) {
+            if (j < j1) {
+                if (j == q) {
+                    tr = 1.0; ov = 0.0;
+                    P.basis[r] = var;
+                    if (iter < P.trace_cap) { P.trace[2 * iter] = r; P.trace[2 * iter + 1] = var; }
+                    F.slotvar[j] = lv; F.qring[lm] = q;
+                    for (int k = 0; k < n; ++k) F.pring[pslot(k) * ld + j] = 0.0;
+                    var = lv;
+                }
+                const double p = tr / piv;
+                prown[j] = p;
+                const double u = ov - fs * p;
+                if (j < C - 1) cm_feed(best, bslot, j, var, u);
+            }
+        } else
         if (j < j1) {
             const double p = tr / piv;
             prown[j] = p;
@@ -687,17 +805,26 @@
     }
     LPX_FS_W(6);
     static_assert(SELP_NT / 64 == 8, "lanes8_min_idx: one entry per wave");
+    if constexpr (CM) {
+        best = cm_wave_min(best, bslot);
+        if (lane == 0) { s_v[t >> 6] = best.v; s_i[t >> 6] = best.i; s_s[t >> 6] = bslot; }
+        __syncthreads();
+        best.v = s_v[lane & 7]; best.i = s_i[lane & 7]; bslot = s_s[lane & 7];
+        best = cm_wave_min(best, bslot);
+    } else {
     best = wave_min_idx(best);
     if (lane == 0) { s_v[t >> 6] = best.v; s_i[t >> 6] = best.i; }
     __syncthreads();
     best.v = s_v[lane & 7]; best.i = s_i[lane & 7];
     best = lanes8_min_idx(best);
+    }
     if (n >= 1 && n <= F.defer - 2) {
-        if (t == 0) { P.part_v[b] = best.v; P.part_i[b] = best.i; }
+        if (t == 0) { P.part_v[b] = best.v; P.part_i[b] = best.i; if constexpr (CM) F.pslot[b] = bslot; }
     } else if (t < 64) {
         if (t == 0) {
             __hip_atomic_store(&P.part_v[b], best.v, __ATOMIC_RELAXED, __HIP_MEMORY_SCOPE_AGENT);
             __hip_atomic_store(&P.part_i[b], best.i, __ATOMIC_RELAXED, __HIP_MEMORY_SCOPE_AGENT);
+            if constexpr (CM) __hip_atomic_store(&F.pslot[b], bslot, __ATOMIC_RELAXED, __HIP_MEMORY_SCOPE_AGENT);
         }
         asm volatile("s_waitcnt vmcnt(0)" ::: "memory");
         int last = 0;
@@ -705,10 +832,14 @@
         last = __builtin_amdgcn_readfirstlane(last);
         if (last) {
             MinIdx x; x.v = __builtin_inf(); x.i = INT_MAX;
+            int xs = -1;
             if (t < nsel) {
                 x.v = __hip_atomic_load(&P.part_v[t], __ATOMIC_RELAXED, __HIP_MEMORY_SCOPE_AGENT);
                 x.i = __hip_atomic_load(&P.part_i[t], __ATOMIC_RELAXED, __HIP_MEMORY_SCOPE_AGENT);
-            }
+                if constexpr (CM) xs = __hip_atomic_load(&F.pslot[t], __ATOMIC_RELAXED, __HIP_MEMORY_SCOPE_AGENT);
+            }
+            if constexpr (CM) { x = cm_wave_min(x, xs); if (x.i != INT_MAX) x.i = xs; }
+            else
             x = wave_min_idx(x);
             if (t == 0) {
                 nxt->qn = (x.i == INT_MAX) ? -1 : x.i;
@@ -718,8 +849,10 @@
     }
     LPX_FS_W(7);
     if (b == 0 && t == 0) {
+        if constexpr (!CM) {
         P.basis[r] = q;
         if (iter < P.trace_cap) { P.trace[2 * iter] = r; P.trace[2 * iter + 1] = q; }
+        }
         F.rring[lm] = r;
         nxt->status = LPX_RUNNING; nxt->iter = iter + 1; nxt->r = r; nxt->q = q;
         nxt->phase = cur.phase; nxt->fdf_count = cur.fdf_count; nxt->dual_iter = cur.dual_iter;
@@ -729,6 +862,14 @@
     }
     LPX_FS_W(8);
     LPX_FS_END(n);
+}
+__global__ __launch_bounds__(SELP_NT) void lpx_pivot_select(FusedParams F, const double* __restrict__ rat, const SelcRec* recs)
+{
+    pivot_select_body<false>(F, rat, recs);
+}
+__global__ __launch_bounds__(SELP_NT) void lpx_pivot_select_cm(FusedParams F, const double* __restrict__ rat, const SelcRec* recs)
+{
+    pivot_select_body<true>(F, rat, recs);
 }
 
 __global__ __launch_bounds__(256) void lpx_pivot_flush(FusedParams F, int buf, int n, int slot0)
@@ -751,6 +892,76 @@
     P.T[(size_t)i * ld + j] = v;
 }
 
+static constexpr int CE_NT = 1024;
+__global__ __launch_bounds__(CE_NT) void lpx_compact_map(CompactIo io, int32_t* cshape, int32_t* caux)
+{
+    __shared__ int s_cnt[CE_NT];
+    const int t = threadIdx.x, nv = io.C - 1, m = io.R - 1;
+    for (int v = t; v < nv; v += CE_NT) io.vmap[v] = 0;
+    if (t == 0) { cshape[0] = io.R; cshape[1] = io.C - io.R + 1; caux[0] = -1; caux[1] = 0; }
+    __syncthreads();
+    for (int k = t; k < m; k += CE_NT) {
+        const int v = io.basis[k];
+        if (v < 0 || v >= nv || atomicCAS(&io.vmap[v], 0, -2 - k) != 0) *io.flag = 1;
+    }
+    __syncthreads();
+    const int per = (nv + CE_NT - 1) / CE_NT, v0 = min(nv, t * per), v1 = min(nv, v0 + per);
+    int cnt = 0;
+    for (int v = v0; v < v1; ++v) cnt += io.vmap[v] == 0;
+    s_cnt[t] = cnt;
+    __syncthreads();
+    if (t == 0) { int run = 0; for (int k = 0; k < CE_NT; ++k) { const int c = s_cnt[k]; s_cnt[k] = run; run += c; } }
+    __syncthreads();
+    int slot = s_cnt[t];
+    for (int v = v0; v < v1; ++v) {
+        if (io.vmap[v] == 0) { io.vmap[v] = slot; io.slotvar[slot] = v; ++slot; }
+    }
+    if (t == 0) { io.vmap[nv] = io.C - io.R; io.slotvar[io.C - io.R] = nv; }
+}
+__global__ __launch_bounds__(256) void lpx_compact_unmap(CompactIo io)
+{
+    const int k = blockIdx.x * 256 + threadIdx.x;
+    if (k <= io.C - io.R) io.vmap[io.slotvar[k]] = k;
+    if (k < io.R - 1) io.vmap[io.basis[k]] = -2 - k;
+}
+__global__ __launch_bounds__(256) void lpx_compact_gather(CompactIo io)
+{
+    const int i = blockIdx.y, v = blockIdx.x * 256 + threadIdx.x;
+    if (i >= io.R || v >= io.C) return;
+    const double x = io.full[(size_t)i * io.ld + v];
+    const int mp = io.vmap[v];
+    if (mp >= 0) {
+        io.comp[(size_t)i * io.cld + mp] = x;
+        if (v == io.C - 1) for (int j = mp + 1; j < io.cld; ++j) io.comp[(size_t)i * io.cld + j] = 0.0;
+    } else {
+        const double want = i == -2 - mp ? 1.0 : 0.0;
+        if (__double_as_longlong(x) != __double_as_longlong(want)) *io.flag = 1;
+    }
+}
+__global__ __launch_bounds__(256) void lpx_compact_exit(FusedParams F, CompactIo io, const double* src, int n, int slot0)
+{
+    const int i = blockIdx.y, v = blockIdx.x * 256 + threadIdx.x;
+    if (i >= io.R || v >= io.ld) return;
+    double x = 0.0;
+    if (v < io.C) {
+        const int mp = io.vmap[v];
+        if (mp < 0) x = i == -2 - mp ? 1.0 : 0.0;
+        else if (mp == F.caux[0]) x = F.fring[(size_t)F.caux[1] * F.P.R + i];
+        else {
+            const size_t cld = (size_t)io.cld, fld = (size_t)F.P.R;
+            const int ring = 2 * F.defer;
+            x = (n == 1 && mp == F.qring[slot0]) ? 0.0 : src[(size_t)i * cld + mp];
+            for (int s = 0; s < n; ++s) {
+                const int sl = slot0 + s < ring ? slot0 + s : slot0 + s - ring;
+                const double pc = F.pring[(size_t)sl * cld + mp];
+                const double nx = x - F.fring[(size_t)sl * fld + i] * pc;
+                x = i == F.rring[sl] ? pc : nx;
+            }
+        }
+    }
+    io.full[(size_t)i * io.ld + v] = x;
+}
+
 int fused_policy(int ld, int R) { return policy_for(tableau_bytes(ld, R), FUSED_CACHED_BYTES); }
 
 hipError_t launch_fused_init(const FusedParams& f, hipStream_t s)
@@ -779,7 +990,15 @@
     const dim3 gc((f.P.R + SELC_ROWS - 1) / SELC_ROWS), gr(f.P.nblk);
     const size_t lds = sizeof(double) * (size_t)f.P.R;
     const SelcRec* recs = reinterpret_cast<const SelcRec*>(rat + selc_rec_offset(f.P.R));
-    if (e0 && e1) {
+    if (f.compact) {
+        if (e0 && e1) {
+            hipExtLaunchKernelGGL(lpx_pivot_ratio_cm, gc, dim3(SELC_ROWS), 0, s, e0, nullptr, 0, f, rat);
+            hipExtLaunchKernelGGL(lpx_pivot_select_cm, gr, dim3(SELP_NT), lds, s, nullptr, e1, 0, f, (const double*)rat, recs);
+        } else {
+            hipLaunchKernelGGL(lpx_pivot_ratio_cm, gc, dim3(SELC_ROWS), 0, s, f, rat);
+            hipLaunchKernelGGL(lpx_pivot_select_cm, gr, dim3(SELP_NT), lds, s, f, (const double*)rat, recs);
+        }
+    } else if (e0 && e1) {
         hipExtLaunchKernelGGL(lpx_pivot_ratio, gc, dim3(SELC_ROWS), 0, s, e0, nullptr, 0, f, rat);
         hipExtLaunchKernelGGL(lpx_pivot_select, gr, dim3(SELP_NT), lds, s, nullptr, e1, 0, f, (const double*)rat, recs);
     } else {
@@ -793,6 +1012,22 @@
 size_t pivot_ratio_bytes(int R) { return selc_ratio_bytes(R); }
 bool pivot_select_is_pair(int ld, int R) { return R <= SELP_LDS_ROWS && tableau_bytes(ld, R) > ((size_t)SELP_MIN_MB << 20); }
 
+static FusedKernel compact_kernel(int d)
+{
+    switch (d) {
+    case 3: return lpx_pivot_fused_cm<3>;
+    case 4: return lpx_pivot_fused_cm<4>;
+    case 8: return lpx_pivot_fused_cm<8>;
+    case 12: return lpx_pivot_fused_cm<12>;
+    case 16: return lpx_pivot_fused_cm<16>;
+    default: return nullptr;
+    }
+}
+bool pivot_compact_ok(int ld, int R, int d)
+{
+    return pivot_select_is_pair(ld, R) && fused_policy(ld, R) != 0 && d >= 3 && compact_kernel(d) != nullptr;
+}
+
 hipError_t launch_pivot_fused(const FusedParams& f0, double* rat, long long L, hipStream_t s, hipEvent_t e0, hipEvent_t e1)
 {
     FusedParams f = f0;
@@ -800,7 +1035,7 @@
     if (d < 1 || d > FP_DMAX) return hipErrorInvalidValue;
     f.lm = (int)(L % (2 * d)); f.par = f.lm & 1;
     const bool sweep = L > 0 && L % d == 0;
-    const int ld = f.P.ld, R = f.P.R;
+    const int ld = f.compact ? f.ld_full : f.P.ld, R = f.P.R;
     if (!sweep) {
         if (pivot_select_is_pair(ld, R)) return rat ? launch_pivot_select_pair(f, rat, s, e0, e1) : hipErrorInvalidValue;
         return launch_pivot_select_ws(f, s, e0, e1);
@@ -808,11 +1043,12 @@
     const int rows = fp_rows(d);
     const int pol = fused_policy(ld, R);
     const int strip = (pol != 0 && d >= 3) ? FP_STRIP_BLOCKS : 1;
-    const int ncw = (ld + 127) / 128, nunits = ncw * (((R + rows - 1) / rows + strip - 1) / strip);
+    const int ncw = (f.P.ld + 127) / 128, nunits = ncw * (((R + rows - 1) / rows + strip - 1) / strip);
     const int nblocks = f.P.nblk + (nunits + (FP_NT / 64) - 1) / (FP_NT / 64);
     int mixmod = pol == 2 ? mixmod_for(tableau_bytes(ld, R)) : 0;
     if (mixmod > 1) mixmod = std::max(1, mixmod * UPDS_ROWS / rows);
-    const FusedKernel kern = pol == 0 ? FusedKernels::c[d - 1] : FusedKernels::nt[d - 1];
+    if (f.compact && !pivot_compact_ok(ld, R, d)) return hipErrorInvalidValue;
+    const FusedKernel kern = f.compact ? compact_kernel(d) : pol == 0 ? FusedKernels::c[d - 1] : FusedKernels::nt[d - 1];
     return launch_k(kern, dim3(nblocks), dim3(FP_NT), 0, s, e0, e1, f, ncw, nunits, mixmod);
 }
 
@@ -823,9 +1059,25 @@
     return hipGetLastError();
 }
 
+hipError_t launch_compact_entry(const CompactIo& io, int32_t* cshape, int32_t* caux, hipStream_t s)
+{
+    hipLaunchKernelGGL(lpx_compact_map, dim3(1), dim3(CE_NT), 0, s, io, cshape, caux);
+    hipLaunchKernelGGL(lpx_compact_gather, dim3((io.C + 255) / 256, io.R), dim3(256), 0, s, io);
+    return hipGetLastError();
+}
+
+hipError_t launch_compact_exit(const FusedParams& f, const CompactIo& io, const double* src, int n, int slot0, hipStream_t s)
+{
+    hipLaunchKernelGGL(lpx_compact_unmap, dim3((std::max(io.R, io.C - io.R + 1) + 255) / 256), dim3(256), 0, s, io);
+    hipLaunchKernelGGL(lpx_compact_exit, dim3((io.ld + 255) / 256, io.R), dim3(256), 0, s, f, io, src, n, slot0);
+    return hipGetLastError();
+}
+
 hipError_t pivot_fused_init()
 {
-    return hipFuncSetAttribute(reinterpret_cast<const void*>(lpx_pivot_select), hipFuncAttributeMaxDynamicSharedMemorySize, 8 * SELP_LDS_ROWS);
+    hipError_t e = hipFuncSetAttribute(reinterpret_cast<const void*>(lpx_pivot_select), hipFuncAttributeMaxDynamicSharedMemorySize, 8 * SELP_LDS_ROWS);
+    if (e != hipSuccess) return e;
+    return hipFuncSetAttribute(reinterpret_cast<const void*>(lpx_pivot_select_cm), hipFuncAttributeMaxDynamicSharedMemorySize, 8 * SELP_LDS_ROWS);
 }
 #ifdef LPX_STAMPS
 hipError_t pivot_fused_stamps(unsigned long long* acc, int clear) { return stamps_take(acc, clear); }
diff --git a/linear_programming_solver_lpr381_amd/csrc/lpx_tableau.cpp b/linear_programming_solver_lpr381_amd/csrc/lpx_tableau.cpp
--- a/linear_programming_solver_lpr381_amd/csrc/lpx_tableau.cpp
+++ b/linear_programming_solver_lpr381_amd/csrc/lpx_tableau.cpp
@@ -151,7 +151,7 @@
     for (hipEvent_t e : t->events) hipEventDestroy(e);
     hipFree(t->T); hipFree(t->slab); hipFree(t->snapT); hipFree(t->snapBasis);
     hipFree(t->frows); hipFree(t->fcols); hipFree(t->fchosen); hipFree(t->cutbuf);
-    hipFree(t->fT); hipFree(t->fslab); hipFree(t->dring);
+    hipFree(t->fT); hipFree(t->fslab); hipFree(t->dring); hipFree(t->cslab);
     hipFree(t->rgws);
     t->bnd.free();
     hipFree(t->xr); hipFree(t->xp); hipFree(t->xgen); hipFree(t->xbasis); hipFree(t->xT); hipFree(t->xc); hipFree(t->xq);
@@ -404,6 +404,20 @@
     return 0;
 }
 
+static constexpr int COMPACT_MIN_SWEEPS = 8;
+static int pivot_compact_env()
+{
+    static const int v = [] { const char* e = std::getenv("LPX_PIVOT_COMPACT"); return e ? (e[0] == '0' ? 0 : 1) : -1; }();
+    return v;
+}
+static bool compact_buffers(lpx_tableau* t)
+{
+    if (t->cslab) return true;
+    const size_t ints = (size_t)t->ld + (size_t)t->Ccap + 128 + 2 * (size_t)pivot_defer_max() + 8;
+    if (malloc_retry((void**)&t->cslab, sizeof(int32_t) * ints) != hipSuccess) { (void)hipGetLastError(); t->cslab = nullptr; return false; }
+    return true;
+}
+
 static int run_fused(lpx_tableau* t, const SelParams& p, const lpx_run_opts* o, lpx_stats* stats, int start_iter)
 {
     const int d = pivot_defer(t->ld, t->Rcap);
@@ -414,6 +428,32 @@
     f.fring = f.pring + (size_t)t->dring_slots * t->ld;
     f.rring = (int32_t*)(f.fring + (size_t)t->dring_slots * t->Rcap);
     f.defer = d;
+    t->last_compact = false;
+    CompactIo io; std::memset(&io, 0, sizeof(io));
+    double pass_ms = 0.0;
+    const int cenv = pivot_compact_env();
+    if (cenv != 0 && pivot_compact_ok(t->ld, t->Rcap, d) && t->C - t->R >= 1
+        && (cenv == 1 || pivot_budget(o, false) >= (long long)COMPACT_MIN_SWEEPS * d) && compact_buffers(t)) {
+        int32_t* ci = (int32_t*)t->cslab;
+        io.full = t->T; io.ld = t->ld; io.R = t->R; io.C = t->C;
+        io.comp = t->fT; io.cld = (t->C - t->R + 1 + 15) / 16 * 16;
+        io.basis = t->basis; io.slotvar = ci; io.vmap = ci + t->ld;
+        int32_t* pslot = io.vmap + t->Ccap; int32_t* qring = pslot + 128; int32_t* caux = qring + 2 * pivot_defer_max();
+        int32_t* cshape = caux + 2; io.flag = cshape + 2;
+        const double t0 = now_ms();
+        int32_t bad = 0;
+        LPX_HIP_TRY(hipMemsetAsync(io.flag, 0, sizeof(int32_t), t->stream));
+        LPX_HIP_TRY(launch_compact_entry(io, cshape, caux, t->stream));
+        LPX_HIP_TRY(hipMemcpyAsync(&bad, io.flag, sizeof(bad), hipMemcpyDeviceToHost, t->stream));
+        LPX_HIP_TRY(hipStreamSynchronize(t->stream));
+        pass_ms += now_ms() - t0;
+        if (!bad) {
+            f.P.T = t->fT; f.T1 = t->T; f.P.ld = io.cld; f.P.C = t->C - t->R + 1; f.P.shape = cshape;
+            f.compact = 1; f.ld_full = t->ld;
+            f.slotvar = io.slotvar; f.pslot = pslot; f.qring = qring; f.caux = caux;
+            t->last_compact = true;
+        }
+    }
     LoopCtx c; DevState init;
     make_ctx(t, p, c, init);
     c.key.assign(reinterpret_cast<const char*>(&f), sizeof(f));
@@ -435,6 +475,14 @@
     LPX_HIP_TRY(hipMemcpy(recs, t->frec, sizeof(recs), hipMemcpyDeviceToHost));
     const DevState& last = recs[1].pad[2] > recs[0].pad[2] ? recs[1] : recs[0];
     const int buf = last.pad[3] & 1, npend = (last.pad[3] >> 1) & 31, slot0 = last.pad[3] >> 8;
+    if (f.compact) {
+        const double t0 = now_ms();
+        io.full = buf ? t->fT : t->T;
+        LPX_HIP_TRY(launch_compact_exit(f, io, buf ? t->T : t->fT, npend, slot0, t->stream));
+        if (buf) LPX_HIP_TRY(hipMemcpyAsync(t->T, t->fT, sizeof(double) * (size_t)t->R * t->ld, hipMemcpyDeviceToDevice, t->stream));
+        LPX_HIP_TRY(hipStreamSynchronize(t->stream));
+        pass_ms += now_ms() - t0;
+    } else
     if (npend > 0) {
         LPX_HIP_TRY(launch_pivot_flush(f, buf, npend, slot0, t->stream));
         LPX_HIP_TRY(hipStreamSynchronize(t->stream));
@@ -443,6 +491,7 @@
         LPX_HIP_TRY(hipMemcpyAsync(t->T, t->fT, sizeof(double) * (size_t)t->R * t->ld, hipMemcpyDeviceToDevice, t->stream));
         LPX_HIP_TRY(hipStreamSynchronize(t->stream));
     }
+    if (stats) stats->loop_ms += pass_ms;
     return rc;
 }
 
@@ -450,12 +499,15 @@
 }
 
 extern "C" {
+
+int lpx_tableau_last_run_compact(const lpx_tableau* t) { return t && t->last_compact ? 1 : 0; }
 
 int lpx_primal_run(lpx_tableau* t, const lpx_run_opts* o, lpx_pivot_cb cb, void* user, lpx_stats* st)
 {
     if (!t) { set_error("lpx_primal_run: null tableau"); return LPX_EINVAL; }
     lpx_run_opts d; if (!o) { lpx_default_opts(&d, 0); o = &d; }
     if (t->R < 2) { set_error("lpx_primal_run: tableau needs at least one constraint row"); return LPX_EINVAL; }
+    t->last_compact = false;
     static const bool res_env = [] { const char* e = std::getenv("LPX_RESIDENT"); return !(e && e[0] == '0'); }();
     int resume = 0;
     if (o->resident > 0 || (o->resident == 0 && res_env && !o->profile && (o->batch == 0 || o->batch >= 32))) {
```

Result: faster. 61280, median of 6 (+14.3%).
